# Ecogenomics/CheckM

Hardware: NVIDIA H100
Metric: genomes/hour (higher is better)
Workload: dtype int16 (SSV) / u8 (MSV) / int16 (Viterbi) / f32 (Forward, domain definition)

## Files before the change

### checkm_b200/_lib.py

```python
import ctypes as C
import os

_HERE = os.path.dirname(os.path.abspath(__file__))
LIB_PATH = os.environ.get("CKM_LIBRARY") or os.path.join(_HERE, "libckm.so")


class ModelInfo(C.Structure):
    _fields_ = [("name", C.c_char * 128), ("acc", C.c_char * 64), ("desc", C.c_char * 256), ("M", C.c_int32),
                ("has_ga", C.c_int32), ("has_tc", C.c_int32), ("has_nc", C.c_int32),
                ("ga", C.c_float * 2), ("tc", C.c_float * 2), ("nc", C.c_float * 2), ("evparam", C.c_float * 6),
                ("ga_d", C.c_double * 2), ("tc_d", C.c_double * 2), ("nc_d", C.c_double * 2)]


class Hit(C.Structure):
    _fields_ = [("bin", C.c_int32), ("seq", C.c_int32), ("model", C.c_int32), ("tlen", C.c_int32), ("qlen", C.c_int32),
                ("dom", C.c_int32), ("ndom", C.c_int32),
                ("hmm_from", C.c_int32), ("hmm_to", C.c_int32), ("ali_from", C.c_int32), ("ali_to", C.c_int32),
                ("env_from", C.c_int32), ("env_to", C.c_int32),
                ("full_score", C.c_float), ("full_bias", C.c_float), ("dom_score", C.c_float), ("dom_bias", C.c_float),
                ("acc", C.c_float),
                ("full_evalue", C.c_double), ("c_evalue", C.c_double), ("i_evalue", C.c_double),
                ("full_lnP", C.c_double), ("dom_lnP", C.c_double)]


class Stats(C.Structure):
    _fields_ = [("n_pairs", C.c_int64), ("n_cells", C.c_int64), ("n_ssv_cand", C.c_int64), ("n_past_msv", C.c_int64),
                ("n_past_bias", C.c_int64), ("n_past_vit", C.c_int64), ("n_past_fwd", C.c_int64),
                ("n_hits_seq", C.c_int64), ("n_domains", C.c_int64), ("n_reported", C.c_int64),
                ("ms_ssv", C.c_float), ("ms_msv", C.c_float), ("ms_bias", C.c_float), ("ms_vit", C.c_float),
                ("ms_fwd", C.c_float), ("ms_domdef", C.c_float), ("ms_total", C.c_float),
                ("kernel_launches", C.c_int64), ("n_vit_redo", C.c_int64), ("n_msv_exact", C.c_int64),
                ("n_queue_retries", C.c_int64)]


class QaRow(C.Structure):
    _fields_ = [("bin", C.c_int32), ("counts", C.c_int32 * 6), ("n_markers", C.c_int32), ("n_sets", C.c_int32),
                ("unique_hits", C.c_int32), ("multi_hits", C.c_int32),
                ("completeness", C.c_double), ("contamination", C.c_double)]


class MarkerHit(C.Structure):
    _fields_ = [("bin", C.c_int32), ("model", C.c_int32), ("seq_a", C.c_int32), ("seq_b", C.c_int32),
                ("target_length", C.c_int32), ("hmm_from", C.c_int32), ("hmm_to", C.c_int32),
                ("ali_from", C.c_int32), ("ali_to", C.c_int32), ("env_from", C.c_int32), ("env_to", C.c_int32),
                ("order", C.c_int32), ("src_row", C.c_int32), ("dict_key", C.c_int64)]


class ReduceOpts(C.Structure):
    _fields_ = [("ignore_thresholds", C.c_int32), ("skip_pseudogene", C.c_int32), ("skip_adjacent", C.c_int32),
                ("individual_markers", C.c_int32), ("evalue_threshold", C.c_double), ("evalue_exp10", C.c_int32),
                ("pad0", C.c_int32), ("evalue_mant", C.c_double), ("length_threshold", C.c_double),
                ("pseudogene_length", C.c_double)]


class ReduceMeta(C.Structure):
    _fields_ = [("is_pfam", C.c_void_p), ("is_tigr", C.c_void_p), ("clan", C.c_void_p),
                ("nest_off", C.c_void_p), ("nest_idx", C.c_void_p), ("has_cut", C.c_void_p), ("cutoffs", C.c_void_p), ("row_scores", C.c_void_p),
                ("scaffold_id", C.c_void_p), ("orf_num", C.c_void_p), ("name_rank", C.c_void_p),
                ("bin_set_off", C.c_void_p), ("set_marker_off", C.c_void_p), ("set_marker_idx", C.c_void_p)]


class BamFilter(C.Structure):
    _fields_ = [("all_reads", C.c_int32), ("min_qc", C.c_int32), ("min_align", C.c_double), ("max_edit", C.c_double)]


class OutlierIn(C.Structure):
    _fields_ = [("nseq", C.c_int64), ("nbins", C.c_int32), ("ntables", C.c_int32), ("bin_off", C.c_void_p),
                ("len", C.c_void_p), ("acgt", C.c_void_p), ("coding", C.c_void_p), ("sig_row", C.c_void_p),
                ("bin_gc_table", C.c_void_p), ("bin_cd_table", C.c_void_p), ("td_table", C.c_int32), ("pad", C.c_int32),
                ("table_off", C.c_void_p), ("table_key", C.c_void_p), ("table_lo", C.c_void_p), ("table_hi", C.c_void_p),
                ("binsig_in", C.c_void_p)]


class OutlierOut(C.Structure):
    _fields_ = [("bin_means", C.c_void_p), ("bin_sig", C.c_void_p), ("seq_values", C.c_void_p), ("seq_mask", C.c_void_p),
                ("kernel_ms", C.c_float * 3)]


SYMBOLS = ["ckm_init", "ckm_destroy", "ckm_last_error", "ckm_version", "ckm_device_name",
           "ckm_models_load", "ckm_models_count", "ckm_models_info", "ckm_models_find", "ckm_models_select",
           "ckm_models_write", "ckm_models_free", "ckm_digitize", "ckm_fasta_parse", "ckm_seqdb_create", "ckm_seqdb_free",
           "ckm_search", "ckm_search_per_bin", "ckm_hits_free", "ckm_align", "ckm_last_stats", "ckm_msv_scores",
           "ckm_filter_scores", "ckm_viterbi_scores", "ckm_write_domtblout", "ckm_reduce", "ckm_genome_check", "ckm_free", "ckm_allgather_qa", "ckm_nccl_unique_id",
           "ckm_nccl_comm_init", "ckm_nccl_comm_destroy", "ckm_fasta_scan_nt", "ckm_scaffold_stats",
           "ckm_kmer_counts", "ckm_kmer_columns", "ckm_format_kmer_profiles", "ckm_merge_pairs", "ckm_format_merger_rows",
           "ckm_bgzf_blocks", "ckm_bgzf_inflate", "ckm_bam_coverage", "ckm_bam_windows",
           "ckm_parse_kmer_profiles", "ckm_sigs_create", "ckm_sigs_free", "ckm_outlier_scores", "ckm_window_stats",
           "ckm_id_join", "ckm_format_unbinned"]

_lib = None


def lib():
    global _lib
    if _lib is not None:
        return _lib
    if not os.path.exists(LIB_PATH):
        raise ImportError("checkm_b200: %s is missing; run `python -c 'import __graft_entry__ as g; g.build()'` "
                          "(there is no CPU fallback)" % LIB_PATH)
    L = C.CDLL(LIB_PATH)
    vp, i32, i64, dbl = C.c_void_p, C.c_int32, C.c_int64, C.c_double
    L.ckm_last_error.restype = C.c_char_p
    L.ckm_version.restype = C.c_char_p
    L.ckm_init.argtypes = [C.c_int, C.POINTER(vp)]
    L.ckm_destroy.argtypes = [vp]
    L.ckm_destroy.restype = None
    L.ckm_device_name.argtypes = [vp, C.c_char_p, C.c_int]
    L.ckm_models_load.argtypes = [vp, C.c_char_p, C.POINTER(vp)]
    L.ckm_models_count.argtypes = [vp]
    L.ckm_models_info.argtypes = [vp, C.c_int, C.POINTER(ModelInfo)]
    L.ckm_models_find.argtypes = [vp, C.c_char_p]
    L.ckm_models_select.argtypes = [vp, C.POINTER(C.c_char_p), C.c_int, vp, C.POINTER(C.c_int)]
    L.ckm_models_write.argtypes = [vp, vp, C.c_int, C.c_char_p]
    L.ckm_models_free.argtypes = [vp]
    L.ckm_models_free.restype = None
    L.ckm_digitize.argtypes = [C.c_char_p, i64, vp]
    L.ckm_fasta_parse.argtypes = [C.c_char_p, i64, vp, vp, i32, vp, i64, C.POINTER(i32), C.POINTER(i64), C.POINTER(i64)]
    L.ckm_fasta_scan_nt.argtypes = [C.c_char_p, i64, vp, i64, vp, vp, i32, vp, i64, C.POINTER(i32), C.POINTER(i64), C.POINTER(i64)]
    L.ckm_scaffold_stats.argtypes = [vp, vp, i64, vp, vp, i32, vp, vp, vp, i64, C.POINTER(i64), C.POINTER(C.c_float)]
    L.ckm_kmer_counts.argtypes = [vp, vp, i64, vp, vp, i32, i32, vp, C.POINTER(C.c_float)]
    L.ckm_kmer_columns.argtypes = [i32, vp]
    L.ckm_format_kmer_profiles.argtypes = [vp, i32, i32, vp, vp, vp, i64, C.POINTER(i64)]
    L.ckm_merge_pairs.argtypes = [vp, vp, i32, i32, vp, dbl, dbl, dbl, dbl, vp, i64, C.POINTER(i64), C.POINTER(C.c_float)]
    L.ckm_format_merger_rows.argtypes = [vp, vp, i32, vp, vp, vp, vp, i64, vp, i64, C.POINTER(i64)]
    L.ckm_parse_kmer_profiles.argtypes = [C.c_char_p, i64, i32, i32, vp, vp, vp, i64, C.POINTER(i64)]
    L.ckm_sigs_create.argtypes = [vp, vp, i64, C.POINTER(vp)]
    L.ckm_sigs_free.argtypes = [vp]
    L.ckm_sigs_free.restype = None
    L.ckm_outlier_scores.argtypes = [vp, vp, C.POINTER(OutlierIn), C.POINTER(OutlierOut)]
    L.ckm_id_join.argtypes = [vp, C.c_char_p, i64, i32, vp, i64, vp, vp, vp, vp, vp, C.POINTER(i64), C.POINTER(i64),
                              C.POINTER(C.c_float)]
    L.ckm_format_unbinned.argtypes = [vp, vp, vp, vp, vp, vp, vp, i64, vp, i64, vp, i64, C.POINTER(i64), C.POINTER(i64)]
    L.ckm_window_stats.argtypes = [vp, vp, i64, vp, vp, i32, i64, vp, vp, vp, vp, C.POINTER(C.c_float)]
    L.ckm_bgzf_blocks.argtypes = [vp, i64, i64, vp, i64, C.POINTER(i64), C.POINTER(i64)]
    L.ckm_bgzf_inflate.argtypes = [vp, vp, i64, i64, vp, i64, vp, i64, C.POINTER(i64), C.POINTER(C.c_float)]
    L.ckm_bam_coverage.argtypes = [vp, vp, i64, i64, vp, i64, vp, vp, i64, i32, C.POINTER(BamFilter), vp, vp, C.POINTER(i64)]
    L.ckm_bam_windows.argtypes = [vp, vp, i64, i64, vp, i64, vp, vp, i64, i32, C.POINTER(BamFilter), vp, i64, vp, vp, vp, vp,
                                  C.POINTER(i64)]
    L.ckm_seqdb_create.argtypes = [vp, vp, vp, i32, vp, i32, C.POINTER(vp)]
    L.ckm_seqdb_free.argtypes = [vp]
    L.ckm_seqdb_free.restype = None
    L.ckm_search.argtypes = [vp, vp, vp, i32, vp, dbl, dbl, C.POINTER(C.POINTER(Hit)), C.POINTER(i64)]
    L.ckm_search_per_bin.argtypes = [vp, vp, vp, vp, vp, dbl, dbl, C.POINTER(C.POINTER(Hit)), C.POINTER(i64)]
    L.ckm_align.argtypes = [vp, vp, i32, vp, vp, vp]
    L.ckm_hits_free.argtypes = [C.POINTER(Hit)]
    L.ckm_hits_free.restype = None
    L.ckm_last_stats.argtypes = [vp, C.POINTER(Stats)]
    L.ckm_msv_scores.argtypes = [vp, vp, vp, i32, vp, vp]
    L.ckm_filter_scores.argtypes = [vp, vp, vp, i32, vp, vp, vp, vp, vp]
    L.ckm_viterbi_scores.argtypes = [vp, vp, vp, i32, vp, i32, vp]
    L.ckm_write_domtblout.argtypes = [vp, C.POINTER(Hit), i64, i32, i32, C.POINTER(C.c_char_p), C.POINTER(C.c_char_p),
                                      C.c_char_p]
    L.ckm_reduce.argtypes = [vp, i32, i32, i32, C.POINTER(Hit), i64, C.POINTER(ReduceOpts), C.POINTER(ReduceMeta),
                             C.POINTER(C.POINTER(QaRow)), C.POINTER(i32), C.POINTER(C.POINTER(MarkerHit)),
                             C.POINTER(i64)]
    L.ckm_genome_check.argtypes = [vp, i32, vp, vp, vp, i32, vp]
    L.ckm_free.argtypes = [vp]
    L.ckm_free.restype = None
    L.ckm_allgather_qa.argtypes = [vp, vp, vp, i32, i32, i32, vp, vp]
    L.ckm_nccl_unique_id.argtypes = [vp, i32]
    L.ckm_nccl_comm_init.argtypes = [vp, i32, i32, vp, C.POINTER(vp)]
    L.ckm_nccl_comm_destroy.argtypes = [vp]
    L.ckm_nccl_comm_destroy.restype = None
    _lib = L
    return L


class CkmError(RuntimeError):
    def __init__(self, code, msg):
        RuntimeError.__init__(self, "libckm error %d: %s" % (code, msg))
        self.code = code


def check(rc):
    if rc != 0:
        raise CkmError(rc, lib().ckm_last_error().decode(errors="replace"))
```

### checkm_b200/csrc/fwdback_blk.cuh

```cuda
#pragma once
#include "device_utils.cuh"
#include "engine.hpp"
#include "fwdback.cuh"

namespace ckm {

constexpr int BLK_LOOKAHEAD_MAXQ = 16;

template <int Q, bool TSMEM>
struct BlkModel {
  int M;
  const float *rfb;
  const float4 *tsm;
  float4 t0[TSMEM ? 1 : Q], t1[TSMEM ? 1 : Q];
  int lane;
  __device__ __forceinline__ float4 T0(int q) const { return TSMEM ? tsm[q * 32 + lane] : t0[TSMEM ? 0 : q]; }
  __device__ __forceinline__ float4 T1(int q) const { return TSMEM ? tsm[(Q + q) * 32 + lane] : t1[TSMEM ? 0 : q]; }
};

template <int Q, bool TSMEM>
__device__ __forceinline__ void blk_model_load(BlkModel<Q, TSMEM> &bm, const ModelScalars &ms, const float4 *tfb, const float *rfb,
                                               float4 *tsm, int lane) {
  bm.M = ms.M; bm.lane = lane;
  bm.rfb = rfb + ms.blk_off * 32 * KPAD + lane;
  bm.tsm = tsm;
  const float4 *src = tfb + ms.blk_off * 32 * 2;
  if (TSMEM) {
    __syncwarp();
    for (int q = 0; q < Q; ++q) { tsm[q * 32 + lane] = __ldg(src + (q * 32 + lane) * 2); tsm[(Q + q) * 32 + lane] = __ldg(src + (q * 32 + lane) * 2 + 1); }
    __syncwarp();
  } else {
#pragma unroll
    for (int q = 0; q < Q; ++q) { bm.t0[TSMEM ? 0 : q] = __ldg(src + (q * 32 + lane) * 2); bm.t1[TSMEM ? 0 : q] = __ldg(src + (q * 32 + lane) * 2 + 1); }
  }
}

template <int Q, bool TSMEM, bool FULL, bool STORE_D = true>
__device__ __forceinline__ float forward_blk(const BlkModel<Q, TSMEM> &bm, const uint8_t *__restrict__ res, int L, const Specials sp,
                                             float *xmx, float *full) {
  const int lane = bm.lane;
  float Mx[Q], Ix[Q], Dx[Q];
#pragma unroll
  for (int q = 0; q < Q; ++q) { Mx[q] = 0.0f; Ix[q] = 0.0f; Dx[q] = 0.0f; }
  if (FULL) {
#pragma unroll
    for (int z = 0; z < 3 * Q; ++z) full[z * 32 + lane] = 0.0f;
  }
  float xE = 0.0f, xN = 1.0f, xJ = 0.0f, xB = sp.nmove, xC = 0.0f, totscale = 0.0f;
  if (xmx != nullptr && lane == 0) { xmx[X_E] = xE; xmx[X_N] = xN; xmx[X_J] = xJ; xmx[X_B] = xB; xmx[X_C] = xC; xmx[X_SCALE] = 1.0f; }
  constexpr bool LA = (Q <= BLK_LOOKAHEAD_MAXQ);
  float ecur[Q];
  int xnext;
  if (LA) {
    const float *rp = bm.rfb + (size_t)((L >= 1) ? __ldg(res) : 0) * Q * 32;
#pragma unroll
    for (int q = 0; q < Q; ++q) ecur[q] = __ldg(rp + q * 32);
    xnext = (L >= 2) ? __ldg(res + 1) : 0;
  } else xnext = (L >= 1) ? __ldg(res) : 0;
  for (int i = 1; i <= L; ++i) {
    float enext[LA ? Q : 1];
    {
      const float *rp = bm.rfb + (size_t)xnext * Q * 32;
      if (LA) {
#pragma unroll
        for (int q = 0; q < Q; ++q) enext[LA ? q : 0] = __ldg(rp + q * 32);
        xnext = (i + 2 <= L) ? __ldg(res + i + 1) : 0;
      } else {
#pragma unroll
        for (int q = 0; q < Q; ++q) ecur[q] = __ldg(rp + q * 32);
        xnext = (i + 1 <= L) ? __ldg(res + i) : 0;
      }
    }
    float pm_in = __shfl_up_sync(0xffffffffu, Mx[Q - 1], 1), pi_in = __shfl_up_sync(0xffffffffu, Ix[Q - 1], 1), pd_in = __shfl_up_sync(0xffffffffu, Dx[Q - 1], 1);
    if (lane == 0) { pm_in = 0.0f; pi_in = 0.0f; pd_in = 0.0f; }
    float md[Q], esum = 0.0f;
#pragma unroll
    for (int q = Q - 1; q >= 0; --q) {
      const float4 t0 = bm.T0(q), t1 = bm.T1(q);
      const float pm = (q > 0) ? Mx[q - 1] : pm_in, pi = (q > 0) ? Ix[q - 1] : pi_in, pd = (q > 0) ? Dx[q - 1] : pd_in;
      float sv = xB * t0.x;
      sv += pm * t0.y;
      sv += pi * t0.z;
      sv += pd * t0.w;
      sv *= ecur[q];
      const float nI = Mx[q] * t1.y + Ix[q] * t1.z;
      md[q] = sv * t1.x;
      Mx[q] = sv; Ix[q] = nI;
      esum += sv;
    }
    float Bb = 0.0f, Tb = 1.0f;
#pragma unroll
    for (int q = 0; q < Q; ++q) { const float tdd = bm.T1(q).w; Bb = md[q] + Bb * tdd; Tb *= tdd; }
    float Bs = Bb, Ts = Tb;
#pragma unroll
    for (int o = 1; o < 32; o <<= 1) {
      const float Bl = __shfl_up_sync(0xffffffffu, Bs, o), Tl = __shfl_up_sync(0xffffffffu, Ts, o);
      if (lane >= o) { Bs = Bs + Bl * Ts; Ts = Ts * Tl; }
    }
    float d = __shfl_up_sync(0xffffffffu, Bs, 1);
    if (lane == 0) d = 0.0f;
#pragma unroll
    for (int q = 0; q < Q; ++q) {
      const bool in = (lane * Q + q + 1) <= bm.M;
      Dx[q] = in ? d : 0.0f;
      esum += Dx[q];
      d = md[q] + d * bm.T1(q).w;
    }
    xE = warp_sum_float(esum);
    xN = xN * sp.nloop;
    xC = (xC * sp.nloop) + (xE * sp.emove);
    xJ = (xJ * sp.nloop) + (xE * sp.eloop);
    xB = (xJ * sp.nmove) + (xN * sp.nmove);
    float scale = 1.0f;
    if (xE > 1.0e4f) {
      scale = xE;
      const float inv = __fdiv_rn(1.0f, xE);
      xN = __fdiv_rn(xN, xE); xC = __fdiv_rn(xC, xE); xJ = __fdiv_rn(xJ, xE); xB = __fdiv_rn(xB, xE);
#pragma unroll
      for (int q = 0; q < Q; ++q) { Mx[q] *= inv; Dx[q] *= inv; Ix[q] *= inv; }
      totscale += (float)log((double)xE);
      xE = 1.0f;
    }
    if (FULL) {
      float *fr = full + (size_t)i * 3 * Q * 32 + lane;
#pragma unroll
      for (int q = 0; q < Q; ++q) { fr[q * 32] = Mx[q]; if (STORE_D) fr[(Q + q) * 32] = Dx[q]; fr[(2 * Q + q) * 32] = Ix[q]; }
    }
    if (xmx != nullptr && lane == 0) {
      float *xr = xmx + (size_t)i * X_NX;
      xr[X_E] = xE; xr[X_N] = xN; xr[X_J] = xJ; xr[X_B] = xB; xr[X_C] = xC; xr[X_SCALE] = scale;
    }
    if (LA) {
#pragma unroll
      for (int q = 0; q < Q; ++q) ecur[q] = enext[LA ? q : 0];
    }
  }
  return totscale + (float)log((double)(xC * sp.nmove));
}

__device__ __forceinline__ void prefetch_l2(const void *p) { asm volatile("prefetch.global.L2 [%0];" ::"l"(p)); }
template <int Q, bool TSMEM, int MODE>
__device__ __forceinline__ void backward_blk(const BlkModel<Q, TSMEM> &bm, const uint8_t *__restrict__ res, int L, const Specials sp,
                                             const float *fxmx, float *bxmx, float *full) {
  const int lane = bm.lane, M = bm.M;
  float Mx[Q], Ix[Q], Dx[Q];
#pragma unroll
  for (int q = 0; q < Q; ++q) { Mx[q] = 0.0f; Ix[q] = 0.0f; Dx[q] = 0.0f; }
  float xC = 0.0f, xE = 0.0f, xJ = 0.0f, xN = 0.0f, xB = 0.0f;
  constexpr bool LA = (Q <= BLK_LOOKAHEAD_MAXQ);
  float ecur[Q];
#pragma unroll
  for (int q = 0; q < Q; ++q) ecur[q] = 0.0f;
  int xnext = (L >= 1) ? __ldg(res + L - 1) : 0;
  for (int i = L; i >= 0; --i) {
    float enext[LA ? Q : 1];
    if (LA) {
      const float *rp = bm.rfb + (size_t)xnext * Q * 32;
#pragma unroll
      for (int q = 0; q < Q; ++q) enext[LA ? q : 0] = __ldg(rp + q * 32);
      xnext = (i >= 2) ? __ldg(res + i - 2) : 0;
    } else if (i < L) {
      const float *rp = bm.rfb + (size_t)xnext * Q * 32;
#pragma unroll
      for (int q = 0; q < Q; ++q) ecur[q] = __ldg(rp + q * 32);
      xnext = (i >= 1) ? __ldg(res + i - 1) : 0;
    }
    if (MODE == 2 && i >= 3) {
      const float *fr = full + (size_t)(i - 2) * 3 * Q * 32;
      if (lane < Q) { prefetch_l2(fr + lane * 32); prefetch_l2(fr + (2 * Q + lane) * 32); }
    }
    float em[Q];
    if (i == L) {
      xC = sp.nmove; xE = xC * sp.emove; xB = 0.0f; xJ = 0.0f; xN = 0.0f;
#pragma unroll
      for (int q = 0; q < Q; ++q) em[q] = 0.0f;
    } else {
      float part = 0.0f;
#pragma unroll
      for (int q = 0; q < Q; ++q) { em[q] = Mx[q] * ecur[q]; part += em[q] * bm.T0(q).x; }
      xB = warp_sum_float(part);
      xC = xC * sp.nloop;
      xJ = (xB * sp.nmove) + (xJ * sp.nloop);
      xN = (xB * sp.nmove) + (xN * sp.nloop);
      xE = (xC * sp.emove) + (xJ * sp.eloop);
    }
    const float s = (i >= 1) ? fxmx[(size_t)i * X_NX + X_SCALE] : 1.0f;
    if (i >= 1) {
      const float inv = (s > 1.0f) ? __fdiv_rn(1.0f, s) : 1.0f;
      float em_next = __shfl_down_sync(0xffffffffu, em[0], 1);
      float4 tn_next;
      {
        const float4 mine = bm.T0(0);
        tn_next.x = 0.0f;
        tn_next.y = __shfl_down_sync(0xffffffffu, mine.y, 1); tn_next.z = __shfl_down_sync(0xffffffffu, mine.z, 1); tn_next.w = __shfl_down_sync(0xffffffffu, mine.w, 1);
      }
      if (lane == 31) { em_next = 0.0f; tn_next.y = 0.0f; tn_next.z = 0.0f; tn_next.w = 0.0f; }
      float cb[Q];
      float Bb = 0.0f, Tb = 1.0f;
#pragma unroll
      for (int q = Q - 1; q >= 0; --q) {
        const int k = lane * Q + q + 1;
        const float mnext = (q < Q - 1) ? em[q + 1] : em_next;
        const float tdm = (q < Q - 1) ? bm.T0(q + 1).w : tn_next.w;
        const bool in = (k <= M);
        cb[q] = in ? (xE + ((k < M) ? mnext * tdm : 0.0f)) : 0.0f;
        const float tdd = in ? bm.T1(q).w : 0.0f;
        Bb = cb[q] + Bb * tdd; Tb *= tdd;
      }
      float Bs = Bb, Ts = Tb;
#pragma unroll
      for (int o = 1; o < 32; o <<= 1) {
        const float Br = __shfl_down_sync(0xffffffffu, Bs, o), Tr = __shfl_down_sync(0xffffffffu, Ts, o);
        if (lane + o < 32) { Bs = Bs + Br * Ts; Ts = Ts * Tr; }
      }
      float dnext = __shfl_down_sync(0xffffffffu, Bs, 1);
      if (lane == 31) dnext = 0.0f;
      float nM[Q], nI[Q], nD[Q];
#pragma unroll
      for (int q = Q - 1; q >= 0; --q) {
        const int k = lane * Q + q + 1;
        const bool in = (k <= M);
        const float4 t1 = bm.T1(q);
        const float mnext = (q < Q - 1) ? em[q + 1] : em_next;
        const float4 tn = (q < Q - 1) ? bm.T0(q + 1) : tn_next;
        const float tmm = (k < M) ? tn.y : 0.0f, tim = (k < M) ? tn.z : 0.0f;
        const float inext = (i < L) ? Ix[q] : 0.0f;
        const float dv = in ? (cb[q] + dnext * t1.w) : 0.0f;
        float mv = xE + mnext * tmm + inext * t1.y + dnext * t1.x;
        float iv = mnext * tim + inext * t1.z;
        if (!in) { mv = 0.0f; iv = 0.0f; }
        nM[q] = mv * inv; nI[q] = iv * inv; nD[q] = dv * inv;
        dnext = dv;
      }
#pragma unroll
      for (int q = 0; q < Q; ++q) { Mx[q] = nM[q]; Ix[q] = nI[q]; Dx[q] = nD[q]; }
      if (s > 1.0f) { xE = __fdiv_rn(xE, s); xN = __fdiv_rn(xN, s); xJ = __fdiv_rn(xJ, s); xB = __fdiv_rn(xB, s); xC = __fdiv_rn(xC, s); }
    } else {
      xC = 0.0f; xJ = 0.0f; xE = 0.0f;
#pragma unroll
      for (int q = 0; q < Q; ++q) { Mx[q] = 0.0f; Ix[q] = 0.0f; Dx[q] = 0.0f; }
    }
    if (MODE == 1) {
      float *fr = full + (size_t)i * 3 * Q * 32 + lane;
#pragma unroll
      for (int q = 0; q < Q; ++q) { fr[q * 32] = Mx[q]; fr[(Q + q) * 32] = Dx[q]; fr[(2 * Q + q) * 32] = Ix[q]; }
    }
    if (MODE == 2 && i >= 1) {
      float *fr = full + (size_t)i * 3 * Q * 32 + lane;
      float fm[Q], fi[Q];
#pragma unroll
      for (int q = 0; q < Q; ++q) { fm[q] = fr[q * 32]; fi[q] = fr[(2 * Q + q) * 32]; }
#pragma unroll
      for (int q = 0; q < Q; ++q) { fr[q * 32] = fm[q] * Mx[q]; fr[(2 * Q + q) * 32] = fi[q] * Ix[q]; }
    }
    if (bxmx != nullptr && lane == 0) {
      float *xr = bxmx + (size_t)i * X_NX;
      xr[X_E] = xE; xr[X_N] = xN; xr[X_J] = xJ; xr[X_B] = xB; xr[X_C] = xC; xr[X_SCALE] = s;
    }
    if (LA) {
#pragma unroll
      for (int q = 0; q < Q; ++q) ecur[q] = enext[LA ? q : 0];
    }
  }
}

}
```

### checkm_b200/csrc/kernels_blk.cu

```cuda
#include "engine.hpp"
#include "device_utils.cuh"
#include "stages.hpp"
#include "fwdback.cuh"
#include "fwdback_blk.cuh"
#include "domdef_common.cuh"
#include "filter_common.cuh"

namespace ckm {

constexpr int BLK_WARPS = 4;

__host__ __device__ constexpr size_t blk_tsm_bytes(int Q) { return (size_t)Q * 32 * 2 * sizeof(float4); }

template <int Q, bool TSMEM>
__global__ void __launch_bounds__(BLK_WARPS * 32) fwd2_kernel(FilterParams p) {
  extern __shared__ __align__(16) uint8_t bsm[];
  const int lane = threadIdx.x & 31, warp = threadIdx.x >> 5;
  float4 *tsm = reinterpret_cast<float4 *>(bsm) + (size_t)warp * Q * 32 * 2;
  const int n = min(*p.in_count, p.in_cap);
  for (int c = blockIdx.x * BLK_WARPS + warp; c < n; c += gridDim.x * BLK_WARPS) {
    Candidate cd = p.in[c];
    const ModelScalars ms = p.ms[cd.model];
    if (ms.vq != Q) continue;
    const int s = cd.seq, L = p.len[s];
    BlkModel<Q, TSMEM> bm;
    blk_model_load<Q, TSMEM>(bm, ms, p.tfb, p.rfb, tsm, lane);
    const float fsc = forward_blk<Q, TSMEM, false>(bm, p.res + p.off[s], L, make_specials(L, true), nullptr, nullptr);
    fwd_verdict(p, cd, fsc, ms, lane);
  }
}

template <int Q, bool TSMEM>
__global__ void __launch_bounds__(BLK_WARPS * 32) regions2_kernel(DomdefParams p) {
  extern __shared__ __align__(16) uint8_t bsm[];
  const int lane = threadIdx.x & 31, warp = threadIdx.x >> 5;
  float4 *tsm = reinterpret_cast<float4 *>(bsm) + (size_t)warp * Q * 32 * 2;
  for (int idx = p.pair_begin + blockIdx.x * BLK_WARPS + warp; idx < p.pair_end; idx += gridDim.x * BLK_WARPS) {
    const int pi = p.pair_order[idx];
    const PairWork pw = p.pairs[pi];
    const ModelScalars ms = p.ms[pw.model];
    if (ms.vq != Q) continue;
    const int L = pw.L;
    BlkModel<Q, TSMEM> bm;
    blk_model_load<Q, TSMEM>(bm, ms, p.tfb, p.rfb, tsm, lane);
    const uint8_t *res = p.res + p.off[pw.seq];
    const Specials sp = make_specials(L, true);
    float *xf = p.xf + pw.row_off * X_NX, *xb = p.xb + pw.row_off * X_NX;
    forward_blk<Q, TSMEM, false>(bm, res, L, sp, xf, nullptr);
    __syncwarp();
    backward_blk<Q, TSMEM, 0>(bm, res, L, sp, xf, xb, nullptr);
    __syncwarp();
    regions_tail(p, pi, L, sp, xf, xb, p.btot + pw.row_off, p.etot + pw.row_off, p.mocc + pw.row_off, p.n2sc + pw.row_off, lane);
    __syncwarp();
  }
}

template <int Q> struct BlockedLayout {
  const float *F; const float4 *tfb; int M;
  static __device__ __forceinline__ int at(int k) { return ((k - 1) % Q) * 32 + (k - 1) / Q; }
  __device__ __forceinline__ float cell(int row, int plane, int k) const { return F[((int64_t)row * 3 + plane) * (Q * 32) + at(k)]; }
  __device__ __forceinline__ float4 t0(int k) const { return __ldg(tfb + at(k) * 2); }
  __device__ __forceinline__ float4 t1(int k) const { return __ldg(tfb + at(k) * 2 + 1); }
  __device__ __forceinline__ void row_best(int row, int lane, float &bm, int &bk, float &bd, int &bdk) const {
    const float *dpc = F + (int64_t)row * 3 * (Q * 32) + lane;
    if constexpr (Q <= 12) {
#pragma unroll
      for (int q = 0; q < Q; ++q) {
        const int kk = lane * Q + q + 1;
        if (kk <= M) {
          const float v = dpc[q * 32]; if (v >= bm) { bm = v; bk = kk; }
          const float w = dpc[(Q + q) * 32]; if (w > bd) { bd = w; bdk = kk; }
        }
      }
    } else {
#pragma unroll 4
      for (int q = 0; q < Q; ++q) {
        const int kk = lane * Q + q + 1;
        if (kk <= M) { const float v = dpc[q * 32]; if (v >= bm) { bm = v; bk = kk; } }
      }
#pragma unroll 4
      for (int q = 0; q < Q; ++q) {
        const int kk = lane * Q + q + 1;
        if (kk <= M) { const float w = dpc[(Q + q) * 32]; if (w > bd) { bd = w; bdk = kk; } }
      }
    }
  }
};

template <int Q, bool TSMEM>
__global__ void __launch_bounds__(BLK_WARPS * 32) envelope2_kernel(DomdefParams p) {
  extern __shared__ __align__(16) uint8_t bsm[];
  const int lane = threadIdx.x & 31, warp = threadIdx.x >> 5;
  float4 *tsm = reinterpret_cast<float4 *>(bsm) + (size_t)warp * Q * 32 * 2;
  float *null2 = reinterpret_cast<float *>(bsm + (TSMEM ? BLK_WARPS * blk_tsm_bytes(Q) : 0)) + warp * 32;
  constexpr int QW = Q * 32;
  for (int idx = p.env_begin + blockIdx.x * BLK_WARPS + warp; idx < p.env_end; idx += gridDim.x * BLK_WARPS) {
    const int ei = p.env_order[idx];
    const Envelope env = p.envs[ei];
    const PairWork pw = p.pairs[env.pair];
    const ModelScalars ms = p.ms[pw.model];
    if (ms.vq != Q) continue;
    BlkModel<Q, TSMEM> bm;
    blk_model_load<Q, TSMEM>(bm, ms, p.tfb, p.rfb, tsm, lane);
    const int M = ms.M, Ld = env.j - env.i + 1;
    const uint8_t *res = p.res + p.off[pw.seq] + (env.i - 1);
    const Specials sp = make_specials(pw.L, false);
    const int64_t mat = (int64_t)(Ld + 1) * 3 * QW;
    float *F = p.scratch + env.scratch_off, *Bm = F;
    float *xf = F + mat, *xb = xf + (int64_t)(Ld + 1) * X_NX, *pps = xb + (int64_t)(Ld + 1) * X_NX;
    float *xo = xf;
    float *n2sc = p.n2sc + pw.row_off;
    const float envsc = forward_blk<Q, TSMEM, true, false>(bm, res, Ld, sp, xf, F);
    __syncwarp();
    backward_blk<Q, TSMEM, 2>(bm, res, Ld, sp, xf, xb, F);
    __syncwarp();
    const float scaleproduct = __fdiv_rn(1.0f, xb[X_N]);
    float em[Q], ein[Q];
#pragma unroll
    for (int q = 0; q < Q; ++q) { em[q] = 0.0f; ein[q] = 0.0f; }
    for (int r = 1; r <= Ld; ++r) {
      if (r + 2 <= Ld && lane < Q) {
        const float *fn = F + (int64_t)(r + 2) * 3 * QW;
        prefetch_l2(fn + lane * 32); prefetch_l2(fn + (2 * Q + lane) * 32);
      }
      const float totr = scaleproduct * xf[(int64_t)r * X_NX + X_SCALE];
      const float *fr = F + (int64_t)r * 3 * QW + lane;
      float vm[Q], vi[Q];
#pragma unroll
      for (int q = 0; q < Q; ++q) { vm[q] = fr[q * 32]; vi[q] = fr[(2 * Q + q) * 32]; }
#pragma unroll
      for (int q = 0; q < Q; ++q) {
        const float pm = vm[q] * totr, pi = vi[q] * totr;
        em[q] = (r == 1) ? pm : em[q] + pm;
        ein[q] = (r == 1) ? pi : ein[q] + pi;
      }
    }
    special_posteriors(sp, xf, xb, scaleproduct, pps, Ld, lane);
    const bool range_err = isinf(scaleproduct);
    if (!range_err && !env.null2_done) {
      const float norm = __fdiv_rn(1.0f, (float)Ld);
      const float xfactor = special_xfactor(pps, Ld, norm, lane);
#pragma unroll
      for (int q = 0; q < Q; ++q) { em[q] *= norm; ein[q] *= norm; }
      for (int x = 0; x < K; ++x) {
        const float *rp = bm.rfb + (size_t)x * QW;
        float part = 0.0f;
#pragma unroll
        for (int q = 0; q < Q; ++q) { part += em[q] * __ldg(rp + q * 32); part += ein[q]; }
        part = warp_sum_float(part);
        if (lane == 0) null2[x] = part + xfactor;
      }
      null2_finish(null2, n2sc, res, env, lane);
    }
    float oasc = 0.0f;
    const float NINF = -INFINITY;
    if (!range_err) {
      float oM[Q], oI[Q], oD[Q];
#pragma unroll
      for (int q = 0; q < Q; ++q) { oM[q] = NINF; oI[q] = NINF; oD[q] = NINF; }
#pragma unroll
      for (int z = 0; z < 3 * Q; ++z) Bm[z * 32 + lane] = NINF;
      OaSpecials os(sp);
      os.store(xo, lane);
      for (int r = 1; r <= Ld; ++r) {
        if (r + 2 <= Ld && lane < Q) {
          const float *fn = F + (int64_t)(r + 2) * 3 * QW;
          prefetch_l2(fn + lane * 32); prefetch_l2(fn + (2 * Q + lane) * 32);
        }
        const float totr = scaleproduct * xf[(int64_t)r * X_NX + X_SCALE];
        const float *ppr = F + (int64_t)r * 3 * QW + lane;
        float *orow = Bm + (int64_t)r * 3 * QW + lane;
        float ppm[Q], ppi[Q];
#pragma unroll
        for (int q = 0; q < Q; ++q) { ppm[q] = ppr[q * 32]; ppi[q] = ppr[(2 * Q + q) * 32]; }
        float pm_in = __shfl_up_sync(0xffffffffu, oM[Q - 1], 1), pi_in = __shfl_up_sync(0xffffffffu, oI[Q - 1], 1), pd_in = __shfl_up_sync(0xffffffffu, oD[Q - 1], 1);
        if (lane == 0) { pm_in = NINF; pi_in = NINF; pd_in = NINF; }
        float a[Q]; bool ps[Q];
        float emax = NINF;
#pragma unroll
        for (int q = Q - 1; q >= 0; --q) {
          const float4 t0 = bm.T0(q), t1 = bm.T1(q);
          const bool in = (lane * Q + q + 1) <= M;
          const float pm = (q > 0) ? oM[q - 1] : pm_in, pi = (q > 0) ? oI[q - 1] : pi_in, pd = (q > 0) ? oD[q - 1] : pd_in;
          float sv = (t0.x > 0.0f) ? os.B : 0.0f;
          sv = fmaxf(sv, (t0.y > 0.0f) ? pm : 0.0f);
          sv = fmaxf(sv, (t0.z > 0.0f) ? pi : 0.0f);
          sv = fmaxf(sv, (t0.w > 0.0f) ? pd : 0.0f);
          sv += ppm[q] * totr;
          if (!in) sv = NINF;
          const float nI = in ? fmaxf((t1.y > 0.0f) ? oM[q] : 0.0f, (t1.z > 0.0f) ? oI[q] : 0.0f) + ppi[q] * totr : NINF;
          a[q] = (t1.x > 0.0f) ? sv : 0.0f;
          ps[q] = (t1.w > 0.0f);
          if (!in) { a[q] = NINF; ps[q] = true; }
          if (!ps[q]) a[q] = fmaxf(a[q], 0.0f);
          oM[q] = sv; oI[q] = nI;
          emax = fmaxf(emax, sv);
        }
        float A = NINF; bool pass = true;
#pragma unroll
        for (int q = 0; q < Q; ++q) { if (ps[q]) { A = fmaxf(a[q], A); } else { A = a[q]; pass = false; } }
        float As = A; bool Ps = pass;
#pragma unroll
        for (int o = 1; o < 32; o <<= 1) {
          const float Al = __shfl_up_sync(0xffffffffu, As, o);
          const int pl = __shfl_up_sync(0xffffffffu, (int)Ps, o);
          if (lane >= o && Ps) { As = fmaxf(As, Al); Ps = (pl != 0); }
        }
        float d = __shfl_up_sync(0xffffffffu, As, 1);
        if (lane == 0) d = NINF;
#pragma unroll
        for (int q = 0; q < Q; ++q) {
          const bool in = (lane * Q + q + 1) <= M;
          oD[q] = in ? d : NINF;
          emax = fmaxf(emax, oD[q]);
          d = ps[q] ? fmaxf(a[q], d) : a[q];
        }
#pragma unroll
        for (int o = 16; o > 0; o >>= 1) emax = fmaxf(emax, __shfl_xor_sync(0xffffffffu, emax, o));
        os.row(sp, pps + r * 3, emax);
#pragma unroll
        for (int q = 0; q < Q; ++q) { orow[q * 32] = oM[q]; orow[(Q + q) * 32] = oD[q]; orow[(2 * Q + q) * 32] = oI[q]; }
        os.store(xo + (int64_t)r * X_NX, lane);
      }
      oasc = os.C;
    }
    __syncwarp();
    OaTrace tr;
    if (!range_err) tr = oa_traceback(BlockedLayout<Q>{Bm, p.tfb + ms.blk_off * 64, M}, p, pw, env, sp, xo, pps, Ld, M, lane);
    write_domain(p, env, n2sc, tr, envsc, oasc, lane);
    __syncwarp();
  }
}

template <class P, class KF>
static int launch_blk(KF kern, const char *name, int Q, bool tsmem, const P &p, int grid, size_t extra, cudaStream_t st) {
  return launch_kernel(kern, name, grid, BLK_WARPS * 32, (tsmem ? BLK_WARPS * blk_tsm_bytes(Q) : 0) + extra, st, p);
}
int launch_fwd2(const FilterParams &p, int cls, int grid, cudaStream_t st) {
  return with_class(cls, [&](auto Q, auto TSMEM) { return launch_blk(fwd2_kernel<Q, TSMEM>, "fwd2_kernel", Q, TSMEM, p, grid, 0, st); });
}
int launch_regions2(const DomdefParams &p, int cls, int grid, cudaStream_t st) {
  return with_class(cls, [&](auto Q, auto TSMEM) { return launch_blk(regions2_kernel<Q, TSMEM>, "regions2_kernel", Q, TSMEM, p, grid, 0, st); });
}
int launch_envelopes2(const DomdefParams &p, int cls, int grid, cudaStream_t st) {
  return with_class(cls, [&](auto Q, auto TSMEM) {
    return launch_blk(envelope2_kernel<Q, TSMEM>, "envelope2_kernel", Q, TSMEM, p, grid, BLK_WARPS * 32 * sizeof(float), st);
  });
}

}
```

### checkm_b200/csrc/kernels_vitp.cu

```cuda
#include "engine.hpp"
#include "device_utils.cuh"
#include "stages.hpp"
#include "filter_common.cuh"

namespace ckm {

constexpr uint32_t VP_FLOORW = 0xD800D800u;
constexpr int      VP_FLOOR  = -10240;
constexpr uint32_t VP_TFLOORW = 0xC000C000u;

__device__ __forceinline__ int vp_lo(uint32_t w) { return (int)(int16_t)(w & 0xffffu); }
__device__ __forceinline__ int vp_hi(uint32_t w) { return (int)w >> 16; }

__global__ void vit_count_kernel(FilterParams p, int32_t *cnt) {
  const int n = min(*p.in_count, p.in_cap);
  for (int i = blockIdx.x * blockDim.x + threadIdx.x; i < n; i += gridDim.x * blockDim.x) {
    const Candidate cd = p.in[i];
    if (!(cd.P > p.F2)) filter_pass(p, cd, 4);
    else if (p.ms[cd.model].vq == 0) vit_redo(p, cd);
    else atomicAdd(cnt + cd.model, 1);
  }
}

__global__ void __launch_bounds__(1024) vit_scan_kernel(FilterParams p, int32_t nmodels, const int32_t *cnt, int32_t *off, int32_t *choff) {
  __shared__ int ws[2][32];
  const int lane = threadIdx.x & 31, warp = threadIdx.x >> 5;
  int run_pairs = 0, run_chunks = 0;
  for (int c = 0; c < N_BLK_CLASSES; ++c) {
    if (threadIdx.x == 0) p.vit_cls_chunks[c] = run_chunks;
    for (int b = 0; b < nmodels; b += 1024) {
      const int m = b + threadIdx.x;
      const int v = (m < nmodels && blk_class(p.ms[m].vq) == c) ? cnt[m] : 0, h = (v + VITP_CHUNK - 1) / VITP_CHUNK;
      int sv = v, sh = h;
#pragma unroll
      for (int o = 1; o < 32; o <<= 1) {
        const int a = __shfl_up_sync(0xffffffffu, sv, o), d = __shfl_up_sync(0xffffffffu, sh, o);
        if (lane >= o) { sv += a; sh += d; }
      }
      if (lane == 31) { ws[0][warp] = sv; ws[1][warp] = sh; }
      __syncthreads();
      if (warp == 0) {
        int tv = ws[0][lane], th = ws[1][lane];
#pragma unroll
        for (int o = 1; o < 32; o <<= 1) {
          const int a = __shfl_up_sync(0xffffffffu, tv, o), d = __shfl_up_sync(0xffffffffu, th, o);
          if (lane >= o) { tv += a; th += d; }
        }
        ws[0][lane] = tv; ws[1][lane] = th;
      }
      __syncthreads();
      if (v > 0) {
        off[m] = run_pairs + (warp ? ws[0][warp - 1] : 0) + sv - v;
        choff[m] = run_chunks + (warp ? ws[1][warp - 1] : 0) + sh - h;
      }
      run_pairs += ws[0][31]; run_chunks += ws[1][31];
      __syncthreads();
    }
  }
  if (threadIdx.x == 0) p.vit_cls_chunks[N_BLK_CLASSES] = run_chunks;
}

__global__ void vit_scatter_kernel(FilterParams p, const int32_t *cnt, int32_t *fill, const int32_t *off, const int32_t *choff) {
  const int n = min(*p.in_count, p.in_cap);
  for (int i = blockIdx.x * blockDim.x + threadIdx.x; i < n; i += gridDim.x * blockDim.x) {
    const int m = p.in[i].model;
    if (!(p.in[i].P > p.F2) || p.ms[m].vq == 0) continue;
    const int r = atomicAdd(fill + m, 1), pos = off[m] + r;
    p.vit_idx[pos] = i;
    if (r % VITP_CHUNK == 0) p.vit_chunks[choff[m] + r / VITP_CHUNK] = make_int2(pos, off[m] + min(r + VITP_CHUNK, cnt[m]));
  }
}

int launch_vit_group(const FilterParams &p, int32_t nmodels, int32_t *ws, int grid, cudaStream_t st) {
  int32_t *cnt = ws, *fill = ws + nmodels, *off = ws + 2 * (size_t)nmodels, *choff = ws + 3 * (size_t)nmodels;
  cudaError_t e = cudaMemsetAsync(ws, 0, sizeof(int32_t) * 2 * (size_t)nmodels, st);
  if (e != cudaSuccess) return cuda_fail(e, "cudaMemsetAsync(vit groups)");
  vit_count_kernel<<<grid, 256, 0, st>>>(p, cnt);
  vit_scan_kernel<<<1, 1024, 0, st>>>(p, nmodels, cnt, off, choff);
  vit_scatter_kernel<<<grid, 256, 0, st>>>(p, cnt, fill, off, choff);
  e = cudaGetLastError();
  return e == cudaSuccess ? CKM_OK : cuda_fail(e, "vit grouping launch");
}

constexpr int VITP_THREADS = 128;

__host__ __device__ constexpr int vitp_smem_bytes(int W, bool tsmem) { return KPAD * W * 32 * 4 + (tsmem ? W * 64 * 16 : 0); }
__host__ __device__ constexpr int vitp_min_blocks(int W) { return W <= 4 ? 4 : (W <= 10 ? 3 : 2); }

template <int W, bool TSMEM>
__global__ void __launch_bounds__(VITP_THREADS, vitp_min_blocks(W)) vitp_kernel(FilterParams p, int cls) {
  extern __shared__ __align__(16) uint4 vsm[];
  __shared__ int s_chunk, s_next;
  __shared__ ModelScalars s_ms;
  uint32_t *esm = reinterpret_cast<uint32_t *>(vsm);
  uint4 *tws = vsm + KPAD * W * 8;
  const int lane = threadIdx.x & 31;
  const uint32_t sel = (lane == 0) ? 0x1054u : 0x3210u;
  const int c0 = p.vit_cls_chunks[cls], nch = p.vit_cls_chunks[cls + 1] - c0;
  for (;;) {
    __syncthreads();
    if (threadIdx.x == 0) {
      const int k = atomicAdd(p.vit_work + cls, 1);
      s_chunk = k;
      if (k < nch) {
        s_next = p.vit_chunks[c0 + k].x;
        s_ms = p.ms[p.in[p.vit_idx[s_next]].model];
      }
    }
    __syncthreads();
    const int k = s_chunk;
    if (k >= nch) break;
    const int2 ch = p.vit_chunks[c0 + k];
    const ModelScalars &ms = s_ms;
    {
      const uint4 *esrc = reinterpret_cast<const uint4 *>(p.rwp + ms.blk_off * 32 * (KPAD / 2));
      for (int z = threadIdx.x; z < KPAD * W * 8; z += VITP_THREADS) vsm[z] = __ldg(esrc + z);
      if (TSMEM) {
        const uint4 *tsrc = p.twp + ms.blk_off * 32;
        for (int z = threadIdx.x; z < W * 64; z += VITP_THREADS) tws[(z & 1) * (W * 32) + (z >> 1)] = __ldg(tsrc + z);
      }
    }
    uint4 tr0[TSMEM ? 1 : W], tr1[TSMEM ? 1 : W];
    if (!TSMEM) {
      const uint4 *tsrc = p.twp + ms.blk_off * 32;
#pragma unroll
      for (int w = 0; w < W; ++w) { tr0[TSMEM ? 0 : w] = __ldg(tsrc + (w * 32 + lane) * 2); tr1[TSMEM ? 0 : w] = __ldg(tsrc + (w * 32 + lane) * 2 + 1); }
    }
#define TR0(w) (TSMEM ? tws[(w) * 32 + lane] : tr0[TSMEM ? 0 : (w)])
#define TR1(w) (TSMEM ? tws[W * 32 + (w) * 32 + lane] : tr1[TSMEM ? 0 : (w)])
    __syncthreads();
    const uint32_t *erow = esm + lane;
    const int ddbound = ms.ddbound_w, cap = 32767 - (int)ms.vit_emax;
    const int e_move = ms.xw_e_move, e_loop = ms.xw_e_loop;
    for (;;) {
      int j = 0;
      if (lane == 0) j = atomicAdd(&s_next, 1);
      j = __shfl_sync(0xffffffffu, j, 0);
      if (j >= ch.y) break;
      const Candidate *cin = p.in + p.vit_idx[j];
      const int s = cin->seq, L = p.len[s];
      bool redo = false;
      const int tmove = p.tmove_w[s];
      const int cost = -tmove - (int)ms.vit_tbm + 64;
      const bool c1 = (cost - (int)ms.xw_e_loop <= 22528) && (cost <= 22240);
      const bool c1p = (cost - (int)ms.xw_e_loop <= 16384);
      redo = !c1;
      float vsc = 0.0f;
      if (!redo) {
        uint32_t Mx[W], Ix[W], Dx[W];
#pragma unroll
        for (int w = 0; w < W; ++w) { Mx[w] = VP_FLOORW; Ix[w] = VP_FLOORW; Dx[w] = VP_FLOORW; }
        int xN = ms.base_w, xB = xN + tmove, xJ = -32768, xC = -32768;
        const uint32_t *rp = reinterpret_cast<const uint32_t *>(p.res + p.off[s]);
        const int nw = (L + 3) >> 2;
        uint32_t wcur = (nw > 0) ? __ldg(rp) : 0u;
        bool stop = false;
        for (int q = 0; q < nw && !stop; ++q) {
          const uint32_t wnext = (q + 1 < nw) ? __ldg(rp + q + 1) : 0u;
#pragma unroll
          for (int rr = 0; rr < 4; ++rr) {
            if (q * 4 + rr >= L) { stop = true; break; }
            const uint32_t *ew = erow + ((wcur >> (8 * rr)) & 0xffu) * (W * 32);
            const uint32_t shM = __shfl_sync(0xffffffffu, Mx[W - 1], (lane + 31) & 31);
            const uint32_t shI = __shfl_sync(0xffffffffu, Ix[W - 1], (lane + 31) & 31);
            const uint32_t shD = __shfl_sync(0xffffffffu, Dx[W - 1], (lane + 31) & 31);
            const uint32_t pm0 = __byte_perm(shM, VP_FLOORW, sel), pi0 = __byte_perm(shI, VP_FLOORW, sel), pd0 = __byte_perm(shD, VP_FLOORW, sel);
            const uint32_t xBw = __byte_perm((uint32_t)xB, 0u, 0x1010u);
            uint32_t md[W];
            uint32_t xEw = VP_FLOORW, dmw = VP_FLOORW;
#pragma unroll
            for (int w = W - 1; w >= 0; --w) {
              const uint32_t pm = (w > 0) ? Mx[w - 1] : pm0, pi = (w > 0) ? Ix[w - 1] : pi0, pd = (w > 0) ? Dx[w - 1] : pd0;
              const uint4 t0 = TR0(w), t1 = TR1(w);
              uint32_t sv = __viaddmax_s16x2(xBw, t0.x, VP_FLOORW);
              sv = __viaddmax_s16x2(pm, t0.y, sv);
              sv = __viaddmax_s16x2(pi, t0.z, sv);
              sv = __viaddmax_s16x2(pd, t0.w, sv);
              sv = __viaddmax_s16x2(sv, ew[w * 32], VP_FLOORW);
              const uint32_t nI = __viaddmax_s16x2(Ix[w], t1.z, __viaddmax_s16x2(Mx[w], t1.y, VP_FLOORW));
              md[w] = __viaddmax_s16x2(sv, t1.x, VP_FLOORW);
              Mx[w] = sv; Ix[w] = nI;
            }
#pragma unroll
            for (int w = 0; w + 1 < W; w += 2) { xEw = __vimax3_s16x2(xEw, Mx[w], Mx[w + 1]); dmw = __vimax3_s16x2(dmw, md[w], md[w + 1]); }
            if (W & 1) { xEw = __vimax3_s16x2(xEw, Mx[W - 1], Mx[W - 1]); dmw = __vimax3_s16x2(dmw, md[W - 1], md[W - 1]); }
            const int xE = __reduce_max_sync(0xffffffffu, max(vp_lo(xEw), vp_hi(xEw)));
            if (xE >= cap) { redo = true; stop = true; break; }
            xC = max(xC, xE + e_move);
            xJ = max(xJ, xE + e_loop);
            xB = max(xJ + tmove, xN + tmove);
            const int Dmax = __reduce_max_sync(0xffffffffu, max(vp_lo(dmw), vp_hi(dmw)));
            if (Dmax + ddbound > xB) {
              if (!c1p) { redo = true; stop = true; break; }
              uint32_t Bb = VP_FLOORW, Tb = 0u;
#pragma unroll
              for (int w = 0; w < W; ++w) { const uint32_t tdd = TR1(w).w; Bb = __viaddmax_s16x2(Bb, tdd, md[w]); Tb = __viaddmax_s16x2(Tb, __vimax3_s16x2(tdd, VP_TFLOORW, VP_TFLOORW), VP_TFLOORW); }
              uint32_t Bs = Bb, Ts = Tb;
#pragma unroll
              for (int o = 1; o < 32; o <<= 1) {
                const uint32_t Bl = __shfl_up_sync(0xffffffffu, Bs, o), Tl = __shfl_up_sync(0xffffffffu, Ts, o);
                if (lane >= o) { Bs = __viaddmax_s16x2(Bl, Ts, Bs); Ts = __viaddmax_s16x2(Ts, Tl, VP_TFLOORW); }
              }
              uint32_t din = __shfl_up_sync(0xffffffffu, Bs, 1), Tex = __shfl_up_sync(0xffffffffu, Ts, 1);
              if (lane == 0) { din = VP_FLOORW; Tex = 0u; }
              const uint32_t lowexit = __shfl_sync(0xffffffffu, Bs, 31);
              const uint32_t dmid = __byte_perm(lowexit, VP_FLOORW, 0x1054u);
              din = __viaddmax_s16x2(dmid, Tex, din);
              uint32_t d = din;
#pragma unroll
              for (int w = 0; w < W; ++w) { Dx[w] = d; d = __viaddmax_s16x2(d, TR1(w).w, md[w]); }
            } else {
              const uint32_t shd = __shfl_sync(0xffffffffu, md[W - 1], (lane + 31) & 31);
#pragma unroll
              for (int w = W - 1; w >= 1; --w) Dx[w] = md[w - 1];
              Dx[0] = __byte_perm(shd, VP_FLOORW, sel);
            }
          }
          wcur = wnext;
        }
        if (!redo && xC <= VP_FLOOR + e_move) redo = true;
        if (!redo) vsc = vit_vsc(xC, tmove, ms);
      }
      Candidate cd = *cin;
      if (redo) {
        if (lane == 0) vit_redo(p, cd);
        continue;
      }
      if (vit_verdict(p, cd, vsc, ms, lane) && lane == 0) filter_pass(p, cd, 4);
    }
#undef TR0
#undef TR1
  }
}

__global__ void all_pairs_kernel(Candidate *out, int32_t *count, const int32_t *slot_model, int32_t nslots, int32_t nseq) {
  const int64_t n = (int64_t)nslots * nseq;
  for (int64_t i = blockIdx.x * (int64_t)blockDim.x + threadIdx.x; i < n; i += (int64_t)gridDim.x * blockDim.x) {
    Candidate cd;
    cd.seq = (int32_t)(i % nseq); cd.model = slot_model[i / nseq]; cd.usc = 0.0f; cd.filtersc = 0.0f; cd.vitsc = 0.0f; cd.fwdsc = 0.0f; cd.P = 1.0;
    out[i] = cd;
  }
  if (blockIdx.x == 0 && threadIdx.x == 0) *count = (int32_t)n;
}
int launch_all_pairs(Candidate *out, int32_t *count, const int32_t *slot_model, int32_t nslots, int32_t nseq, cudaStream_t st) {
  return launch_kernel(all_pairs_kernel, "all_pairs_kernel", 592, 256, 0, st, out, count, slot_model, nslots, nseq);
}

int launch_vitp(const FilterParams &p, int cls, int grid, cudaStream_t st) {
  return with_class(cls, [&](auto Q, auto TSMEM) {
    return launch_kernel(vitp_kernel<Q / 2, TSMEM>, "vitp_kernel", grid, VITP_THREADS, vitp_smem_bytes(Q / 2, TSMEM), st, p, cls);
  });
}

}
```

### checkm_b200/csrc/search.cu

```cuda
#include <algorithm>
#include <atomic>
#include <chrono>
#include <cstdio>
#include <cmath>
#include <cstdlib>
#include <cstring>
#include <memory>
#include <vector>
#include "engine.hpp"
#include "stages.hpp"
#include "pool.hpp"

using namespace ckm;

namespace ckm {

std::atomic<int> g_live_engines{0};
thread_local ckm_engine *g_pool_engine = nullptr;
thread_local int g_pool_next = 0;
constexpr int X_NX_HOST = 6;
struct EnsembleJob;
int ensembles_launch(ckm_engine *e, const ckm_models *m, DomdefParams &p, const std::vector<PairWork> &pairs,
                     const std::vector<Region> &regs, const std::vector<int> &multi_idx, const std::vector<EnsembleCaps> &caps,
                     cudaStream_t st, EnsembleJob **job_out);
int ensembles_collect(EnsembleJob *job, cudaStream_t st, std::vector<std::vector<Envelope>> &out, std::vector<EnsembleCaps> &grow, int *n_over);
void ensembles_abandon(EnsembleJob *job, cudaStream_t st);
enum { CTR_UNIT4 = 0, CTR_UNIT8, CTR_UNIT16, CTR_UNIT32, CTR_CAND, CTR_MSV, CTR_BIAS, CTR_VIT, CTR_FWD, CTR_ENV, CTR_DOM, CTR_VREDO, CTR_SSVRES, CTR_VWORK = 16 , CTR_N = 32 };
enum { EV_SSV = 0, EV_MSV, EV_BIAS, EV_VIT, EV_FWD, EV_CASCADE_END, EV_DOMDEF, EV_END, EV_CALL };

static int64_t env_scratch_budget() {
  if (const char *v = std::getenv("CKM_ENV_SCRATCH_MB")) {
    char *end = nullptr;
    const long long mb = std::strtoll(v, &end, 10);
    if (end != v && *end == '\0' && mb > 0) return (int64_t)std::min<long long>(mb, (long long)1 << 30) * ((int64_t)1 << 20) / (int64_t)sizeof(float);
  }
  size_t free_b = 0, total_b = 0;
  cudaMemGetInfo(&free_b, &total_b);
  const size_t neng = (size_t)std::max(1, g_live_engines.load());
  return (int64_t)std::min<size_t>(total_b * 4 / 10 / neng, (size_t)56 << 30) / (int64_t)sizeof(float);
}
struct SearchKnobs { bool blk, vitp, ssv_resolve, trace; int ens_first; int64_t env_budget; };
static SearchKnobs read_knobs(bool envelopes) {
  auto starts = [](const char *name, char c) { const char *v = std::getenv(name); return v != nullptr && v[0] == c; };
  SearchKnobs k;
  k.blk = !starts("CKM_BLK", '0');
  k.vitp = k.blk && !starts("CKM_VITP", '0');
  k.ssv_resolve = !starts("CKM_SSV_RESOLVE", '0');
  k.trace = starts("CKM_TRACE", '1');
  const char *ens = std::getenv("CKM_ENS_FIRST");
  k.ens_first = ens == nullptr ? -1 : (ens[0] == '0' ? 0 : 1);
  k.env_budget = envelopes ? env_scratch_budget() : 0;
  return k;
}
struct Trace {
  bool on; std::chrono::steady_clock::time_point t0, last;
  explicit Trace(bool on_) : on(on_) { t0 = last = std::chrono::steady_clock::now(); }
  void mark(const char *what) {
    if (!on) return;
    const auto now = std::chrono::steady_clock::now();
    std::fprintf(stderr, "[ckm trace] %-28s +%8.3f ms  (%9.3f)\n", what, std::chrono::duration<double, std::milli>(now - last).count(),
                 std::chrono::duration<double, std::milli>(now - t0).count());
    last = now;
  }
};

static int cls_of(int M, bool use_blk) { return use_blk ? blk_class(vq_of(M)) : N_BLK_CLASSES; }

static int fan_out(ckm_engine *e) {
  CKM_CUDA(cudaEventRecord(e->fan_ev, e->stream));
  for (auto &s : e->cls) CKM_CUDA(cudaStreamWaitEvent(s, e->fan_ev, 0));
  return CKM_OK;
}
static int fan_in(ckm_engine *e) {
  for (int c = 0; c < ckm_engine::NCLS; ++c) {
    CKM_CUDA(cudaEventRecord(e->cls_ev[c], e->cls[c]));
    CKM_CUDA(cudaStreamWaitEvent(e->stream, e->cls_ev[c], 0));
  }
  return CKM_OK;
}

template <class P> static int per_class(ckm_engine *e, const P &p, int (*blocked)(const P &, int, int, cudaStream_t), int blk_per_sm,
                                        int (*unblocked)(const P &, int, cudaStream_t), int per_sm, bool widest_first = false) {
  const int nsm = e->prop.multiProcessorCount;
  int rc;
  if ((rc = fan_out(e))) return rc;
  for (int i = 0; i < ckm_engine::NCLS; ++i) {
    const int c = widest_first ? ckm_engine::NCLS - 1 - i : i;
    if (c == N_BLK_CLASSES) rc = unblocked ? unblocked(p, nsm * per_sm, e->cls[c]) : CKM_OK;
    else rc = p.use_blk ? blocked(p, c, nsm * blk_per_sm, e->cls[c]) : CKM_OK;
    if (rc) return rc;
  }
  return fan_in(e);
}
template <class Launch> static int launch_class_runs(ckm_engine *e, const std::vector<int32_t> &order, const std::vector<int8_t> &cls, size_t b0, size_t b1, Launch launch) {
  const int nsm = e->prop.multiProcessorCount;
  int rc;
  if ((rc = fan_out(e))) return rc;
  while (b0 < b1) {
    size_t r1 = b0; const int c = cls[order[b0]];
    while (r1 < b1 && cls[order[r1]] == c) ++r1;
    const int cnt = (int)(r1 - b0);
    const int grid = c < N_BLK_CLASSES ? std::min(nsm * 8, (cnt + 3) / 4) : std::min(nsm * 4, (cnt + FWD_WARPS - 1) / FWD_WARPS);
    if ((rc = launch(c, (int32_t)b0, (int32_t)r1, grid, e->cls[c]))) return rc;
    e->stats.kernel_launches++;
    b0 = r1;
  }
  return CKM_OK;
}

struct ActiveMasks { DevBuf tile_active, model_active, model_slot; bool all_active = true; };
static FilterParams filter_params(const ckm_models *m, const ckm_seqdb *db, ActiveMasks &am) {
  FilterParams p{};
  p.res = db->d_res; p.off = db->d_off; p.len = db->d_len; p.lenA = db->d_lenA; p.lenB = db->d_lenB; p.tmove_w = db->d_tmove_w;
  p.ms = m->d_scalars; p.bias_eo = m->d_bias_eo; p.rwv = m->d_rwv; p.twv = m->d_twv; p.rfv = m->d_rfv; p.tfv = m->d_tfv;
  p.twb = m->d_twb; p.rwb = m->d_rwb; p.tfb = m->d_tfb; p.rfb = m->d_rfb; p.twp = m->d_twp; p.rwp = m->d_rwp;
  p.row_elems = ((m->maxM + 31) / 32) * 32 + 64;
  p.F1 = 0.02; p.F2 = 1e-3; p.F3 = 1e-5;
  p.model_slot = am.model_slot.as<int32_t>(); p.nseq = db->nseq;
  return p;
}

static DomdefParams domdef_params(const ckm_models *m, const ckm_seqdb *db, const SearchKnobs &k) {
  DomdefParams p{};
  p.res = db->d_res; p.off = db->d_off; p.nullsc = db->d_nullsc; p.ms = m->d_scalars; p.rfv = m->d_rfv; p.tfv = m->d_tfv;
  p.row_elems = ((m->maxM + 31) / 32) * 32 + 64;
  p.tfb = m->d_tfb; p.rfb = m->d_rfb; p.use_blk = k.blk ? 1 : 0;
  return p;
}
static void fill_filter_stats(ckm_engine *e, int64_t n_pairs, const int32_t *ctr, unsigned long long cells, int stages) {
  ckm_stats &s = e->stats;
  s.n_pairs = n_pairs; s.n_cells = (int64_t)cells;
  s.n_ssv_cand = (int64_t)ctr[CTR_CAND] + ctr[CTR_SSVRES]; s.n_msv_exact = ctr[CTR_CAND]; s.n_past_msv = ctr[CTR_MSV]; s.n_past_bias = ctr[CTR_BIAS];
  s.n_past_vit = ctr[CTR_VIT]; s.n_past_fwd = ctr[CTR_FWD]; s.n_vit_redo = ctr[CTR_VREDO];
  float *ms[] = {&s.ms_ssv, &s.ms_msv, &s.ms_bias, &s.ms_vit, &s.ms_fwd};
  for (int i = 0; i < stages; ++i) cudaEventElapsedTime(ms[i], e->ev[EV_SSV + i], e->ev[EV_SSV + i + 1]);
}
static std::vector<float> &logsum_table() {
  static std::vector<float> t = [] {
    std::vector<float> v(16000);
    for (int i = 0; i < 16000; ++i) v[i] = (float)std::log(1.0 + std::exp((double)-i / 1000.0));
    return v;
  }();
  return t;
}

static int build_masks(const ckm_models *m, const ckm_seqdb *db, const int32_t *model_idx, int32_t nmodels,
                       const int64_t *bin_model_offsets, ActiveMasks &am, std::vector<int32_t> &slot_of_model, cudaStream_t st) {
  const int ndb = (int)m->models.size(), nbins = db->nbins, ntiles = (int)m->tiles.size();
  slot_of_model.assign(ndb, -1);
  bool all = (bin_model_offsets == nullptr) && (model_idx == nullptr || nmodels == ndb);
  if (model_idx == nullptr) { for (int i = 0; i < ndb; ++i) slot_of_model[i] = i; }
  else if (bin_model_offsets == nullptr) {
    for (int i = 0; i < nmodels; ++i) {
      if (model_idx[i] < 0 || model_idx[i] >= ndb) { set_error("model index out of range"); return CKM_EINVAL; }
      if (slot_of_model[model_idx[i]] >= 0) { set_error("duplicate model index in query list"); return CKM_EINVAL; }
      slot_of_model[model_idx[i]] = i;
    }
    if (all) for (int i = 0; i < ndb; ++i) if (slot_of_model[i] < 0) all = false;
  }
  am.all_active = all;
  int rc;
  if ((rc = am.model_slot.alloc(sizeof(int32_t) * ndb))) return rc;
  CKM_CUDA(cudaMemcpyAsync(am.model_slot.p, slot_of_model.data(), sizeof(int32_t) * ndb, cudaMemcpyHostToDevice, st));
  if (all) return CKM_OK;
  std::vector<uint8_t> ma((size_t)nbins * ndb, 0), ta((size_t)nbins * ntiles, 0);
  for (int b = 0; b < nbins; ++b) {
    if (bin_model_offsets == nullptr) {
      for (int i = 0; i < nmodels; ++i) ma[(size_t)b * ndb + model_idx[i]] = 1;
    } else {
      for (int64_t i = bin_model_offsets[b]; i < bin_model_offsets[b + 1]; ++i) {
        if (model_idx[i] < 0 || model_idx[i] >= ndb) { set_error("model index out of range"); return CKM_EINVAL; }
        if (ma[(size_t)b * ndb + model_idx[i]]) { set_error("duplicate model index in the query list of bin " + std::to_string(b)); return CKM_EINVAL; }
        ma[(size_t)b * ndb + model_idx[i]] = 1;
      }
    }
    for (int t = 0; t < ntiles; ++t) {
      const TileDesc &td = m->tiles[t];
      uint8_t any = 0;
      for (int j = 0; j < td.nmodels; ++j) any |= ma[(size_t)b * ndb + m->tile_models[td.first_model + j].model];
      ta[(size_t)b * ntiles + t] = any;
    }
  }
  if ((rc = am.model_active.alloc(ma.size()))) return rc;
  if ((rc = am.tile_active.alloc(ta.size()))) return rc;
  CKM_CUDA(cudaMemcpyAsync(am.model_active.p, ma.data(), ma.size(), cudaMemcpyHostToDevice, st));
  CKM_CUDA(cudaMemcpyAsync(am.tile_active.p, ta.data(), ta.size(), cudaMemcpyHostToDevice, st));
  CKM_CUDA(cudaStreamSynchronize(st));
  return CKM_OK;
}
struct Stage1 {
  DevBuf cand, pass, bnd, glist, cells;
  int32_t cand_cap = 0, pass_cap = 0;
};
constexpr int64_t QUEUE_MAX = (int64_t)1 << 30;
constexpr int QUEUE_ATTEMPTS = 3;
static int32_t queue_cap(int64_t n_pairs, int64_t divisor, int attempt) {
  int64_t want = n_pairs / divisor + 65536;
  for (int a = 0; a < attempt && want < n_pairs; ++a) want *= 8;
  return (int32_t)std::min<int64_t>(std::min<int64_t>(n_pairs, QUEUE_MAX), std::max<int64_t>((int64_t)1 << 16, want));
}

static int run_stage1(ckm_engine *e, const SearchKnobs &k, const ckm_models *m, const ckm_seqdb *db, ActiveMasks &am, int64_t n_pairs,
                      Stage1 &s1, int32_t *xj_dense, int attempt = 0) {
  cudaStream_t st = e->stream;
  int rc;
  s1.cand_cap = queue_cap(n_pairs, 6, attempt);
  const int64_t n_bypass = (int64_t)m->ssv_bypass.size() * db->nseq;
  s1.cand_cap = (int32_t)std::min<int64_t>(QUEUE_MAX, (int64_t)s1.cand_cap + n_bypass);
  s1.pass_cap = queue_cap(n_pairs, 12, attempt);
  if ((rc = s1.cand.alloc(sizeof(int2) * (size_t)s1.cand_cap))) return rc;
  if ((rc = s1.pass.alloc(sizeof(Candidate) * (size_t)s1.pass_cap))) return rc;
  if ((rc = s1.cells.alloc(sizeof(unsigned long long)))) return rc;
  CKM_CUDA(cudaMemsetAsync(e->d_counters, 0, CTR_N * sizeof(int32_t), st));
  CKM_CUDA(cudaMemsetAsync(s1.cells.p, 0, sizeof(unsigned long long), st));
  const int nsm = e->prop.multiProcessorCount;
  bool need_bnd = false;
  for (int nt : m->chain_ntiles) need_bnd |= (nt > 1);
  const int64_t bnd_stride = ((int64_t)db->maxL + 31) / 16 * 16;
  if (need_bnd) { if ((rc = s1.bnd.alloc((size_t)nsm * SSV_WARPS_HOST * 2 * bnd_stride * sizeof(int16_t)))) return rc; }
  std::vector<int32_t> gl[4];
  for (size_t g = 0; g < m->groups.size(); ++g) gl[m->groups[g].J == 4 ? 0 : (m->groups[g].J == 8 ? 1 : (m->groups[g].J == 16 ? 2 : 3))].push_back((int32_t)g);
  std::vector<int32_t> flat;
  size_t goff[4];
  for (int c = 0; c < 4; ++c) { goff[c] = flat.size(); flat.insert(flat.end(), gl[c].begin(), gl[c].end()); }
  if ((rc = s1.glist.alloc(sizeof(int32_t) * std::max<size_t>(flat.size(), 1)))) return rc;
  if (!flat.empty()) CKM_CUDA(cudaMemcpyAsync(s1.glist.p, flat.data(), sizeof(int32_t) * flat.size(), cudaMemcpyHostToDevice, st));
  CKM_CUDA(cudaStreamSynchronize(st));

  CKM_CUDA(cudaEventRecord(e->ev[EV_SSV], st));
  SsvParams sp{};
  sp.res = db->d_res; sp.off = db->d_off; sp.len = db->d_len; sp.bin = db->d_bin;
  sp.msvB = db->d_msvB; sp.tjb = db->d_tjb; sp.order = db->d_order;
  sp.nseq = db->nseq; sp.seq_chunk = 128; sp.nchunks = (db->nseq + sp.seq_chunk - 1) / sp.seq_chunk;
  sp.groups = m->d_groups; sp.tiles = m->d_tiles; sp.tile_models = m->d_tile_models; sp.tile_blob = m->d_tile_blob;
  sp.chain_first_tile = m->d_chain_first_tile; sp.chain_ntiles = m->d_chain_ntiles;
  sp.tile_active = am.all_active ? nullptr : am.tile_active.as<uint8_t>();
  sp.model_active = am.all_active ? nullptr : am.model_active.as<uint8_t>();
  sp.ntiles = (int32_t)m->tiles.size(); sp.nmodels = (int32_t)m->models.size();
  sp.cand = s1.cand.as<int2>(); sp.cand_count = e->d_counters + CTR_CAND; sp.cand_cap = s1.cand_cap;
  sp.bnd = need_bnd ? s1.bnd.as<int16_t>() : nullptr; sp.bnd_stride = bnd_stride;
  sp.cells = s1.cells.as<unsigned long long>();
  sp.resolve = k.ssv_resolve ? 1 : 0;
  sp.ms = m->d_scalars; sp.nullsc = db->d_nullsc;
  sp.pass = s1.pass.as<Candidate>(); sp.pass_count = e->d_counters + CTR_MSV; sp.pass_cap = s1.pass_cap;
  sp.resolved_count = e->d_counters + CTR_SSVRES;
  sp.xj_dense = xj_dense; sp.model_slot = am.model_slot.as<int32_t>();
  sp.F1 = 0.02;
  const int Js[4] = {4, 8, 16, 32};
  for (int c = 0; c < 4; ++c) {
    if (gl[c].empty() || db->nseq == 0) continue;
    sp.group_list = s1.glist.as<int32_t>() + goff[c]; sp.ngroups = (int32_t)gl[c].size();
    sp.unit_counter = e->d_counters + CTR_UNIT4 + c;
    int64_t maxbytes = 0;
    for (int g : gl[c]) maxbytes = std::max<int64_t>(maxbytes, m->groups[g].table_bytes);
    const int64_t units = (int64_t)sp.ngroups * sp.nchunks;
    const int grid = (int)std::min<int64_t>(nsm, units);
    if ((rc = launch_ssv(Js[c], sp, grid, (size_t)maxbytes, st))) return rc;
    e->stats.kernel_launches++;
  }
  if (!m->ssv_bypass.empty()) {
    if ((rc = launch_ssv_bypass(m->d_ssv_bypass, (int32_t)m->ssv_bypass.size(), db->nseq, db->d_len, db->d_bin,
                                am.all_active ? nullptr : am.model_active.as<uint8_t>(), (int32_t)m->models.size(),
                                s1.cand.as<int2>(), e->d_counters + CTR_CAND, s1.cand_cap, st))) return rc;
    e->stats.kernel_launches++;
  }
  CKM_CUDA(cudaEventRecord(e->ev[EV_MSV], st));
  MsvParams p{};
  p.res = db->d_res; p.off = db->d_off; p.len = db->d_len; p.nullsc = db->d_nullsc; p.tjb = db->d_tjb;
  p.ms = m->d_scalars; p.rbv = m->d_rbv; p.rmb = m->d_rmb;
  p.cand = s1.cand.as<int2>(); p.cand_count = e->d_counters + CTR_CAND; p.cand_cap = s1.cand_cap;
  p.out = s1.pass.as<Candidate>(); p.out_count = e->d_counters + CTR_MSV; p.out_cap = s1.pass_cap;
  p.xj_dense = xj_dense; p.model_slot = am.model_slot.as<int32_t>(); p.nseq = db->nseq;
  p.row_bytes = (m->maxM + 2 + 15) / 16 * 16;
  p.F1 = 0.02;
  p.use_blk = k.blk ? 1 : 0;
  if ((rc = per_class(e, p, launch_msv2, 16, launch_msv_exact, 4))) return rc;
  e->stats.kernel_launches += 1 + (p.use_blk ? N_BLK_CLASSES : 0);
  CKM_CUDA(cudaEventRecord(e->ev[EV_BIAS], st));
  return CKM_OK;
}

static int run_viterbi(ckm_engine *e, const ckm_models *m, FilterParams &p, bool packed, DevBuf &grp) {
  int rc;
  if (packed) {
    const int nm = (int)m->models.size();
    const size_t nchunks = (size_t)p.in_cap / VITP_CHUNK + nm + 1;
    const size_t words = 4 * (size_t)nm + 16 + ((size_t)p.in_cap + 1) / 2 * 2;
    if ((rc = grp.alloc(sizeof(int32_t) * words + sizeof(int2) * nchunks))) return rc;
    int32_t *ws = grp.as<int32_t>();
    p.vit_cls_chunks = ws + 4 * (size_t)nm;
    p.vit_idx = p.vit_cls_chunks + 16;
    p.vit_chunks = reinterpret_cast<int2 *>(ws + words);
    p.vit_work = e->d_counters + CTR_VWORK;
    if ((rc = launch_vit_group(p, nm, ws, e->prop.multiProcessorCount * 8, e->stream))) return rc;
    if ((rc = per_class<FilterParams>(e, p, launch_vitp, 8, nullptr, 0))) return rc;
    e->stats.kernel_launches += 3;
    p.in = p.redo; p.in_count = p.redo_count; p.in_cap = p.redo_cap;
  }
  return per_class(e, p, launch_vit2, 8, launch_vit, 4);
}
struct Stage2 {
  DevBuf a, b, redo, vgrp;
  int32_t cap = 0;
};
static int run_stage2(ckm_engine *e, const SearchKnobs &k, const ckm_models *m, const ckm_seqdb *db, ActiveMasks &am, Stage1 &s1, Stage2 &s2,
                      float *d_filtersc, float *d_vit, float *d_fwd, uint8_t *d_passed) {
  cudaStream_t st = e->stream;
  int rc;
  s2.cap = s1.pass_cap;
  if ((rc = s2.a.alloc(sizeof(Candidate) * (size_t)s2.cap))) return rc;
  if ((rc = s2.b.alloc(sizeof(Candidate) * (size_t)s2.cap))) return rc;
  if ((rc = s2.redo.alloc(sizeof(Candidate) * (size_t)s2.cap))) return rc;
  const int nsm = e->prop.multiProcessorCount;
  FilterParams p = filter_params(m, db, am);
  p.redo = s2.redo.as<Candidate>(); p.redo_count = e->d_counters + CTR_VREDO; p.redo_cap = s2.cap;
  p.use_blk = k.blk ? 1 : 0;
  p.dense_filtersc = d_filtersc; p.dense_vit = d_vit; p.dense_fwd = d_fwd; p.dense_passed = d_passed;
  p.in = s1.pass.as<Candidate>(); p.in_count = e->d_counters + CTR_MSV; p.in_cap = s1.pass_cap;
  p.out = s2.a.as<Candidate>(); p.out_count = e->d_counters + CTR_BIAS; p.out_cap = s2.cap;
  if ((rc = launch_bias(p, nsm * 8, st))) return rc;
  CKM_CUDA(cudaEventRecord(e->ev[EV_VIT], st));
  p.in = s2.a.as<Candidate>(); p.in_count = e->d_counters + CTR_BIAS; p.in_cap = s2.cap;
  p.out = s2.b.as<Candidate>(); p.out_count = e->d_counters + CTR_VIT; p.out_cap = s2.cap;
  if ((rc = run_viterbi(e, m, p, k.vitp, s2.vgrp))) return rc;
  CKM_CUDA(cudaEventRecord(e->ev[EV_FWD], st));
  p.in = s2.b.as<Candidate>(); p.in_count = e->d_counters + CTR_VIT; p.in_cap = s2.cap;
  p.out = s2.a.as<Candidate>(); p.out_count = e->d_counters + CTR_FWD; p.out_cap = s2.cap;
  if ((rc = per_class(e, p, launch_fwd2, 8, launch_fwd, 4, true))) return rc;
  CKM_CUDA(cudaEventRecord(e->ev[EV_CASCADE_END], st));
  e->stats.kernel_launches += 3 + (k.vitp ? N_BLK_CLASSES : 0) + (p.use_blk ? 2 * N_BLK_CLASSES : 0);
  return CKM_OK;
}

static int64_t envelope_need(const ckm_models *m, const PairWork &pw, const Envelope &en, bool use_blk) {
  const int64_t Ld = en.j - en.i + 1, Mpad = ((m->models[pw.model].M + 1) + 31) / 32 * 32 + 32;
  const int64_t vq = use_blk ? vq_of(m->models[pw.model].M) : 0;
  const int64_t width = vq ? 32 * vq : Mpad;
  return (vq ? 1 : 2) * (Ld + 1) * 3 * width + (Ld + 1) * 15 + 64;
}
static int run_envelope_waves(ckm_engine *e, const ckm_models *m, const std::vector<PairWork> &pairs, DomdefParams &p, int64_t budget,
                              DevBuf &scratch, std::vector<Envelope> &ev, DevBuf &d_ev, DevBuf &d_ord, bool leave_last) {
  if (ev.empty()) return CKM_OK;
  cudaStream_t st = e->stream;
  int rc;
  std::vector<int64_t> need(ev.size());
  std::vector<int8_t> ecls(ev.size());
  for (size_t i = 0; i < ev.size(); ++i) {
    const PairWork &pw = pairs[ev[i].pair];
    need[i] = envelope_need(m, pw, ev[i], p.use_blk != 0);
    ecls[i] = (int8_t)cls_of(m->models[pw.model].M, p.use_blk != 0);
  }
  budget = std::max<int64_t>(budget, *std::max_element(need.begin(), need.end()));
  if ((rc = d_ev.alloc(sizeof(Envelope) * ev.size())) || (rc = d_ord.alloc(sizeof(int32_t) * ev.size()))) return rc;
  std::vector<int32_t> eorder(ev.size());
  for (size_t w0 = 0, w1; w0 < ev.size(); w0 = w1) {
    int64_t tot = 0;
    for (w1 = w0; w1 < ev.size() && (w1 == w0 || tot + need[w1] <= budget); ++w1) { ev[w1].scratch_off = tot; tot += need[w1]; }
    if (sizeof(float) * (size_t)tot > scratch.bytes && (rc = scratch.alloc(sizeof(float) * (size_t)tot))) return rc;
    for (size_t i = w0; i < w1; ++i) eorder[i] = (int32_t)i;
    std::stable_sort(eorder.begin() + w0, eorder.begin() + w1, [&](int32_t a, int32_t b) { return ecls[a] != ecls[b] ? ecls[a] > ecls[b] : need[a] > need[b]; });
    CKM_CUDA(cudaMemcpyAsync(d_ev.as<Envelope>() + w0, ev.data() + w0, sizeof(Envelope) * (w1 - w0), cudaMemcpyHostToDevice, st));
    CKM_CUDA(cudaMemcpyAsync(d_ord.as<int32_t>() + w0, eorder.data() + w0, sizeof(int32_t) * (w1 - w0), cudaMemcpyHostToDevice, st));
    p.envs = d_ev.as<Envelope>(); p.env_order = d_ord.as<int32_t>(); p.scratch = scratch.as<float>();
    if ((rc = launch_class_runs(e, eorder, ecls, w0, w1, [&](int c, int32_t b0, int32_t b1, int grid, cudaStream_t s) -> int {
          p.env_begin = b0; p.env_end = b1; return c < N_BLK_CLASSES ? launch_envelopes2(p, c, grid, s) : launch_envelopes(p, grid, s); }))) return rc;
    CKM_CUDA(cudaStreamSynchronize(st));
    if (w1 < ev.size() || !leave_last) { if ((rc = fan_in(e))) return rc; CKM_CUDA(cudaStreamSynchronize(st)); }
  }
  return CKM_OK;
}

struct QueryPlan { ActiveMasks am; bool per_bin = false; std::vector<std::vector<int32_t>> qorder; int64_t n_pairs = 0; };
static int plan_queries(const ckm_models *m, const ckm_seqdb *db, const int32_t *model_idx, int32_t nmodels, const int64_t *bin_model_offsets, QueryPlan &q, cudaStream_t st) {
  const int ndb = (int)m->models.size();
  if (model_idx == nullptr && bin_model_offsets == nullptr) nmodels = ndb;
  std::vector<int32_t> slot;
  int rc = build_masks(m, db, model_idx, nmodels, bin_model_offsets, q.am, slot, st);
  if (rc) return rc;
  q.per_bin = bin_model_offsets != nullptr;
  if (q.per_bin) {
    q.qorder.assign(db->nbins, std::vector<int32_t>(ndb, -1));
    for (int b = 0; b < db->nbins; ++b) {
      for (int64_t i = bin_model_offsets[b]; i < bin_model_offsets[b + 1]; ++i) q.qorder[b][model_idx[i]] = (int32_t)(i - bin_model_offsets[b]);
      q.n_pairs += (int64_t)db->bin_nseq[b] * (bin_model_offsets[b + 1] - bin_model_offsets[b]);
    }
  } else {
    q.qorder.emplace_back(std::move(slot));
    q.n_pairs = (int64_t)db->nseq * nmodels;
  }
  return CKM_OK;
}

static int run_cascade(ckm_engine *e, const SearchKnobs &k, const ckm_models *m, const ckm_seqdb *db, ActiveMasks &am, int64_t n_pairs, Stage1 &s1, Stage2 &s2, int32_t *ctr) {
  cudaStream_t st = e->stream;
  unsigned long long cells = 0;
  int rc;
  for (int attempt = 0; attempt < QUEUE_ATTEMPTS; ++attempt) {
    if (attempt > 0) e->stats.n_queue_retries++;
    if ((rc = run_stage1(e, k, m, db, am, std::max<int64_t>(n_pairs, 1), s1, nullptr, attempt))) return rc;
    if ((rc = run_stage2(e, k, m, db, am, s1, s2, nullptr, nullptr, nullptr, nullptr))) return rc;
    CKM_CUDA(cudaMemcpyAsync(ctr, e->d_counters, sizeof(int32_t) * CTR_N, cudaMemcpyDeviceToHost, st));
    CKM_CUDA(cudaMemcpyAsync(&cells, s1.cells.p, sizeof(cells), cudaMemcpyDeviceToHost, st));
    CKM_CUDA(cudaStreamSynchronize(st));
    const bool over = ctr[CTR_CAND] > s1.cand_cap || ctr[CTR_MSV] > s1.pass_cap || ctr[CTR_BIAS] > s2.cap || ctr[CTR_VIT] > s2.cap || ctr[CTR_FWD] > s2.cap ||
                      ctr[CTR_VREDO] > s2.cap;
    if (!over) { fill_filter_stats(e, n_pairs, ctr, cells, 5); return CKM_OK; }
    if (s1.cand_cap >= std::min<int64_t>(n_pairs, QUEUE_MAX) && s1.pass_cap >= std::min<int64_t>(n_pairs, QUEUE_MAX)) break;
  }
  set_error("candidate queue overflow in the filter cascade: more than 2^30 candidate pairs in one batch; search fewer bins per call");
  return CKM_ECAPACITY;
}

static int sorted_pairs(const ckm_seqdb *db, const Candidate *d_fwd_list, int npairs, std::vector<PairWork> &pairs, int64_t &rows) {
  std::vector<Candidate> fl((size_t)npairs);
  if (npairs) CKM_CUDA(cudaMemcpy(fl.data(), d_fwd_list, sizeof(Candidate) * fl.size(), cudaMemcpyDeviceToHost));
  std::sort(fl.begin(), fl.end(), [](const Candidate &a, const Candidate &b) { return a.seq != b.seq ? a.seq < b.seq : a.model < b.model; });
  pairs.assign((size_t)npairs, PairWork{});
  rows = 0;
  for (int i = 0; i < npairs; ++i) {
    PairWork &pw = pairs[i];
    pw.seq = fl[i].seq; pw.model = fl[i].model; pw.L = db->len[pw.seq];
    pw.first_dom = 0; pw.ndom_slots = 0; pw.fwdsc = fl[i].fwdsc; pw.filtersc = fl[i].filtersc; pw.usc = fl[i].usc;
    pw.row_off = rows; rows += pw.L + 1;
  }
  return CKM_OK;
}
struct DomainStage {
  DomdefParams p{};
  DevBuf dpairs, dxf, dxb, dvec, dtbl, dregions, dporder, ddoms, dhits, dscratch, denvs, deorder, denvs2, deorder2;
  std::vector<Region> regs;
  std::vector<DomainOut> doms; std::vector<HitOut> hout;
};
static int run_regions(ckm_engine *e, const SearchKnobs &k, const ckm_models *m, const ckm_seqdb *db, const std::vector<PairWork> &pairs, int64_t rows, DomainStage &D, Trace &tr) {
  cudaStream_t st = e->stream;
  const int npairs = (int)pairs.size();
  const size_t rws = (size_t)std::max<int64_t>(rows, 1);
  int rc;
  if ((rc = D.dpairs.alloc(sizeof(PairWork) * pairs.size())) || (rc = D.dxf.alloc(sizeof(float) * rws * X_NX_HOST)) || (rc = D.dxb.alloc(sizeof(float) * rws * X_NX_HOST)) ||
      (rc = D.dvec.alloc(sizeof(float) * rws * 4)) || (rc = D.dtbl.alloc(sizeof(float) * 16000))) return rc;
  const int region_cap = npairs * 8 + 1024;
  if ((rc = D.dregions.alloc(sizeof(Region) * (size_t)region_cap))) return rc;
  CKM_CUDA(cudaMemcpyAsync(D.dpairs.p, pairs.data(), sizeof(PairWork) * pairs.size(), cudaMemcpyHostToDevice, st));
  CKM_CUDA(cudaMemcpyAsync(D.dtbl.p, logsum_table().data(), sizeof(float) * 16000, cudaMemcpyHostToDevice, st));
  CKM_CUDA(cudaMemsetAsync(e->d_counters + CTR_ENV, 0, sizeof(int32_t), st));
  DomdefParams &p = D.p = domdef_params(m, db, k);
  p.pairs = D.dpairs.as<PairWork>(); p.npairs = npairs;
  p.xf = D.dxf.as<float>(); p.xb = D.dxb.as<float>();
  p.btot = D.dvec.as<float>(); p.etot = p.btot + rws; p.mocc = p.etot + rws; p.n2sc = p.mocc + rws;
  p.regions = D.dregions.as<Region>(); p.region_count = e->d_counters + CTR_ENV; p.region_cap = region_cap;
  p.logsum_tbl = D.dtbl.as<float>();
  std::vector<int32_t> order((size_t)npairs);
  std::vector<int8_t> pcls((size_t)npairs);
  for (int i = 0; i < npairs; ++i) { order[i] = i; pcls[i] = (int8_t)cls_of(m->models[pairs[i].model].M, p.use_blk != 0); }
  std::stable_sort(order.begin(), order.end(), [&](int32_t a, int32_t b) { return pcls[a] != pcls[b] ? pcls[a] > pcls[b] : pairs[a].L > pairs[b].L; });
  if ((rc = D.dporder.alloc(sizeof(int32_t) * order.size()))) return rc;
  CKM_CUDA(cudaMemcpyAsync(D.dporder.p, order.data(), sizeof(int32_t) * order.size(), cudaMemcpyHostToDevice, st));
  p.pair_order = D.dporder.as<int32_t>();
  if ((rc = launch_class_runs(e, order, pcls, 0, (size_t)npairs, [&](int c, int32_t b0, int32_t b1, int grid, cudaStream_t s) -> int {
        p.pair_begin = b0; p.pair_end = b1; return c < N_BLK_CLASSES ? launch_regions2(p, c, grid, s) : launch_regions(p, grid, s); }))) return rc;
  if ((rc = fan_in(e))) return rc;
  int32_t nreg = 0;
  CKM_CUDA(cudaMemcpyAsync(&nreg, e->d_counters + CTR_ENV, sizeof(int32_t), cudaMemcpyDeviceToHost, st));
  CKM_CUDA(cudaStreamSynchronize(st));
  tr.mark("regions kernels");
  if (nreg > region_cap) { set_error("region queue overflow"); return CKM_ECAPACITY; }
  D.regs.resize((size_t)nreg);
  if (nreg) CKM_CUDA(cudaMemcpy(D.regs.data(), D.dregions.p, sizeof(Region) * D.regs.size(), cudaMemcpyDeviceToHost));
  std::sort(D.regs.begin(), D.regs.end(), [](const Region &a, const Region &b) { return a.pair != b.pair ? a.pair < b.pair : a.i < b.i; });
  tr.mark("regions sorted");
  return CKM_OK;
}

struct AbandonJob { cudaStream_t st; void operator()(EnsembleJob *job) const { ensembles_abandon(job, st); } };
static int domain_pass(ckm_engine *e, const SearchKnobs &k, const ckm_models *m, std::vector<PairWork> &pairs, DomainStage &D,
                       const std::vector<int> &multi_idx, std::vector<EnsembleCaps> &caps, Trace &tr, bool *grown) {
  cudaStream_t st = e->stream;
  DomdefParams &p = D.p;
  const std::vector<Region> &regs = D.regs; const int nreg = (int)regs.size();
  int rc;
  *grown = false;
  std::vector<int32_t> reg_slot((size_t)nreg);
  std::vector<Envelope> envs1, envs2;
  int32_t nslots = 0;
  for (auto &pw : pairs) { pw.ndom_slots = 0; pw.first_dom = 0; }
  for (int r = 0, mi = 0; r < nreg; ++r) {
    PairWork &pw = pairs[regs[r].pair];
    if (pw.ndom_slots == 0) pw.first_dom = nslots;
    reg_slot[r] = nslots;
    if (!regs[r].multi) { Envelope en{}; en.pair = regs[r].pair; en.i = regs[r].i; en.j = regs[r].j; en.slot = nslots; envs1.push_back(en); }
    const int n = regs[r].multi ? caps[mi++].envelopes : 1;
    nslots += n; pw.ndom_slots += n;
  }
  D.doms.assign((size_t)nslots, DomainOut{});
  if (nslots == 0) return CKM_OK;
  if ((rc = D.ddoms.alloc(sizeof(DomainOut) * (size_t)nslots)) || (rc = D.dhits.alloc(sizeof(HitOut) * pairs.size()))) return rc;
  CKM_CUDA(cudaMemsetAsync(D.ddoms.p, 0, sizeof(DomainOut) * (size_t)nslots, st));
  CKM_CUDA(cudaMemcpyAsync(D.dpairs.p, pairs.data(), sizeof(PairWork) * pairs.size(), cudaMemcpyHostToDevice, st));
  p.doms = D.ddoms.as<DomainOut>();
  const bool multi = !multi_idx.empty();
  bool ens_first = (k.ens_first == 1);
  if (k.ens_first < 0 && multi) {
    int64_t tot = 0;
    for (const Envelope &en : envs1) tot += envelope_need(m, pairs[en.pair], en, p.use_blk != 0);
    ens_first = tot > k.env_budget;
  }
  std::unique_ptr<EnsembleJob, AbandonJob> ens(nullptr, AbandonJob{e->aux});
  auto launch_ensemble = [&]() -> int {
    CKM_CUDA(cudaEventRecord(e->fan_ev, st));
    CKM_CUDA(cudaStreamWaitEvent(e->aux, e->fan_ev, 0));
    EnsembleJob *job = nullptr;
    const int r = ensembles_launch(e, m, p, pairs, regs, multi_idx, caps, e->aux, &job);
    ens.reset(job);
    return r;
  };
  if (multi && ens_first && (rc = launch_ensemble())) return rc;
  if ((rc = run_envelope_waves(e, m, pairs, p, k.env_budget, D.dscratch, envs1, D.denvs, D.deorder, multi))) return rc;
  tr.mark("envelope batch 1 launched");
  if (multi) {
    if (!ens_first && (rc = launch_ensemble())) return rc;
    if (!envs1.empty()) { if ((rc = fan_in(e))) return rc; CKM_CUDA(cudaStreamSynchronize(st)); }
    std::vector<std::vector<Envelope>> multi_envs; std::vector<EnsembleCaps> grow;
    int n_over = 0;
    if ((rc = ensembles_collect(ens.release(), e->aux, multi_envs, grow, &n_over))) return rc;
    tr.mark("batch 1 + ensemble done");
    if (n_over > 0) {
      for (size_t mi = 0; mi < caps.size(); ++mi) if (grow[mi].segments) caps[mi] = grow[mi];
      *grown = true;
      return CKM_OK;
    }
    for (size_t mi = 0; mi < multi_idx.size(); ++mi) {
      int c = 0;
      for (Envelope en : multi_envs[mi]) { en.slot = reg_slot[multi_idx[mi]] + c++; envs2.push_back(en); }
    }
    if ((rc = run_envelope_waves(e, m, pairs, p, k.env_budget, D.dscratch, envs2, D.denvs2, D.deorder2, false))) return rc;
    tr.mark("envelope batch 2 done");
  }
  p.hits = D.dhits.as<HitOut>();
  if ((rc = launch_scores(p, ((int)pairs.size() + 127) / 128, st))) return rc;
  e->stats.kernel_launches++;
  CKM_CUDA(cudaMemcpyAsync(D.doms.data(), D.ddoms.p, sizeof(DomainOut) * D.doms.size(), cudaMemcpyDeviceToHost, st));
  CKM_CUDA(cudaMemcpyAsync(D.hout.data(), D.dhits.p, sizeof(HitOut) * D.hout.size(), cudaMemcpyDeviceToHost, st));
  CKM_CUDA(cudaStreamSynchronize(st));
  return CKM_OK;
}
constexpr int DOMAIN_PASSES = 4;
static int run_domain_phase(ckm_engine *e, const SearchKnobs &k, const ckm_models *m, std::vector<PairWork> &pairs, DomainStage &D, Trace &tr) {
  std::vector<int> multi_idx;
  for (int r = 0; r < (int)D.regs.size(); ++r) if (D.regs[r].multi) multi_idx.push_back(r);
  std::vector<EnsembleCaps> caps(multi_idx.size(), ENS_DEFAULT_CAPS);
  D.hout.assign(pairs.size(), HitOut{});
  for (int pass = 0; pass < DOMAIN_PASSES; ++pass) {
    if (pass > 0) e->stats.n_queue_retries++;
    bool grown = false;
    int rc = domain_pass(e, k, m, pairs, D, multi_idx, caps, tr, &grown);
    if (rc || !grown) return rc;
  }
  set_error("a multi-domain region keeps outgrowing the capacities it asked for");
  return CKM_ECAPACITY;
}

static std::vector<ckm_hit> assemble_rows(ckm_engine *e, const ckm_models *m, const ckm_seqdb *db, const QueryPlan &q, const std::vector<PairWork> &pairs,
                                          const std::vector<HitOut> &hout, const std::vector<DomainOut> &doms, double Ecut, double domEcut) {
  struct Key { int bin, q, pair; double lnP; int seq; };
  std::vector<Key> keys;
  for (int i = 0; i < (int)pairs.size(); ++i) {
    if (!hout[i].valid) continue;
    const int b = db->bin_of_seq[pairs[i].seq];
    keys.push_back(Key{b, (q.per_bin ? q.qorder[b] : q.qorder[0])[pairs[i].model], i, hout[i].lnP, pairs[i].seq});
  }
  std::sort(keys.begin(), keys.end(), [](const Key &a, const Key &b) {
    if (a.bin != b.bin) return a.bin < b.bin;
    if (a.q != b.q) return a.q < b.q;
    if (a.lnP != b.lnP) return a.lnP < b.lnP;
    return a.seq < b.seq;
  });
  std::vector<ckm_hit> rows_out;
  size_t g0 = 0;
  int64_t n_dom = 0;
  for (size_t i = 0; i < doms.size(); ++i) if (doms[i].ok) n_dom++;
  while (g0 < keys.size()) {
    size_t g1 = g0;
    while (g1 < keys.size() && keys[g1].bin == keys[g0].bin && keys[g1].q == keys[g0].q) ++g1;
    const double Z = (double)db->bin_nseq[keys[g0].bin];
    double domZ = 0.0;
    for (size_t k = g0; k < g1; ++k) if (std::exp(keys[k].lnP) * Z <= Ecut) domZ += 1.0;
    for (size_t k = g0; k < g1; ++k) {
      if (!(std::exp(keys[k].lnP) * Z <= Ecut)) continue;
      const PairWork &pw = pairs[keys[k].pair];
      const HitOut &h = hout[keys[k].pair];
      int nrep = 0;
      for (int d = pw.first_dom; d < pw.first_dom + pw.ndom_slots; ++d)
        if (doms[d].ok && std::exp(doms[d].lnP) * domZ <= domEcut) nrep++;
      int nd = 0;
      for (int d = pw.first_dom; d < pw.first_dom + pw.ndom_slots; ++d) {
        const DomainOut &dm = doms[d];
        if (!dm.ok || !(std::exp(dm.lnP) * domZ <= domEcut)) continue;
        ckm_hit r;
        std::memset(&r, 0, sizeof(r));
        r.bin = keys[k].bin; r.seq = pw.seq; r.model = pw.model; r.tlen = pw.L; r.qlen = m->models[pw.model].M;
        r.dom = ++nd; r.ndom = nrep;
        r.hmm_from = dm.hmmfrom; r.hmm_to = dm.hmmto; r.ali_from = dm.sqfrom; r.ali_to = dm.sqto; r.env_from = dm.ienv; r.env_to = dm.jenv;
        r.full_score = h.score; r.full_bias = h.pre_score - h.score;
        r.dom_score = dm.bitscore; r.dom_bias = (float)((double)dm.dombias * 1.44269504088896341);
        r.acc = (float)(dm.oasc / (1.0 + std::fabs((float)(dm.jenv - dm.ienv))));
        r.full_evalue = std::exp(h.lnP) * Z; r.c_evalue = std::exp(dm.lnP) * domZ; r.i_evalue = std::exp(dm.lnP) * Z;
        r.full_lnP = h.lnP; r.dom_lnP = dm.lnP;
        rows_out.push_back(r);
      }
    }
    g0 = g1;
  }
  e->stats.n_hits_seq = (int64_t)keys.size(); e->stats.n_domains = n_dom; e->stats.n_reported = (int64_t)rows_out.size();
  return rows_out;
}

static int do_search(ckm_engine *e, const SearchKnobs &k, const ckm_models *m, const int32_t *model_idx, int32_t nmodels,
                     const int64_t *bin_model_offsets, const ckm_seqdb *db, double Ecut, double domEcut, ckm_hit **hits_out, int64_t *nhits_out) {
  cudaStream_t st = e->stream;
  *hits_out = nullptr; *nhits_out = 0;
  PoolScope pool_scope(e);
  QueryPlan q;
  int rc = plan_queries(m, db, model_idx, nmodels, bin_model_offsets, q, st);
  if (rc) return rc;
  std::memset(&e->stats, 0, sizeof(e->stats));
  if (q.n_pairs > ((int64_t)1 << 40)) { set_error("ckm_search: more than 2^40 (ORF x HMM) pairs in one call; search fewer bins per call"); return CKM_ECAPACITY; }
  CKM_CUDA(cudaEventRecord(e->ev[EV_CALL], st));
  Trace tr(k.trace);
  Stage1 s1; Stage2 s2; int32_t ctr[CTR_N];
  if ((rc = run_cascade(e, k, m, db, q.am, q.n_pairs, s1, s2, ctr))) return rc;
  tr.mark("filters done");
  std::vector<PairWork> pairs; int64_t rows = 0;
  if ((rc = sorted_pairs(db, s2.a.as<Candidate>(), ctr[CTR_FWD], pairs, rows))) return rc;
  CKM_CUDA(cudaEventRecord(e->ev[EV_DOMDEF], st));
  tr.mark("pair list sorted");
  DomainStage D;
  if (!pairs.empty()) {
    if ((rc = run_regions(e, k, m, db, pairs, rows, D, tr))) return rc;
    if ((rc = run_domain_phase(e, k, m, pairs, D, tr))) return rc;
  }
  CKM_CUDA(cudaEventRecord(e->ev[EV_END], st));
  CKM_CUDA(cudaEventSynchronize(e->ev[EV_END]));
  tr.mark("scores + downloads");
  const std::vector<ckm_hit> rows_out = assemble_rows(e, m, db, q, pairs, D.hout, D.doms, Ecut, domEcut);
  tr.mark("rows assembled");
  cudaEventElapsedTime(&e->stats.ms_domdef, e->ev[EV_DOMDEF], e->ev[EV_END]);
  cudaEventElapsedTime(&e->stats.ms_total, e->ev[EV_CALL], e->ev[EV_END]);
  if (!rows_out.empty()) {
    ckm_hit *out = (ckm_hit *)std::malloc(sizeof(ckm_hit) * rows_out.size());
    if (!out) { set_error("out of host memory"); return CKM_ENOMEM; }
    std::memcpy(out, rows_out.data(), sizeof(ckm_hit) * rows_out.size());
    *hits_out = out;
  }
  *nhits_out = (int64_t)rows_out.size();
  return CKM_OK;
}

static int align_pass(ckm_engine *e, const SearchKnobs &k, const ckm_models *m, const ckm_seqdb *db, std::vector<PairWork> &pairs,
                      std::vector<Envelope> &envs, int64_t rows, std::vector<int32_t> &trace, std::vector<DomainOut> &doms) {
  cudaStream_t st = e->stream;
  PoolScope pool_scope(e);
  DevBuf dpairs, dn2, dtrace, ddoms, dscratch, denvs, deorder;
  int rc;
  const size_t rws = (size_t)rows;
  if ((rc = dpairs.alloc(sizeof(PairWork) * pairs.size())) || (rc = dn2.alloc(sizeof(float) * rws)) || (rc = dtrace.alloc(sizeof(int32_t) * rws)) ||
      (rc = ddoms.alloc(sizeof(DomainOut) * pairs.size()))) return rc;
  CKM_CUDA(cudaMemcpyAsync(dpairs.p, pairs.data(), sizeof(PairWork) * pairs.size(), cudaMemcpyHostToDevice, st));
  CKM_CUDA(cudaMemsetAsync(dn2.p, 0, sizeof(float) * rws, st));
  CKM_CUDA(cudaMemsetAsync(dtrace.p, 0, sizeof(int32_t) * rws, st));
  CKM_CUDA(cudaMemsetAsync(ddoms.p, 0, sizeof(DomainOut) * pairs.size(), st));
  DomdefParams p = domdef_params(m, db, k);
  p.pairs = dpairs.as<PairWork>(); p.npairs = (int32_t)pairs.size();
  p.n2sc = dn2.as<float>(); p.trace = dtrace.as<int32_t>();
  p.doms = ddoms.as<DomainOut>();
  if ((rc = run_envelope_waves(e, m, pairs, p, k.env_budget, dscratch, envs, denvs, deorder, false))) return rc;
  trace.resize(rws);
  doms.resize(pairs.size());
  CKM_CUDA(cudaMemcpyAsync(trace.data(), dtrace.p, sizeof(int32_t) * rws, cudaMemcpyDeviceToHost, st));
  CKM_CUDA(cudaMemcpyAsync(doms.data(), ddoms.p, sizeof(DomainOut) * doms.size(), cudaMemcpyDeviceToHost, st));
  CKM_CUDA(cudaStreamSynchronize(st));
  return CKM_OK;
}

static int do_align(ckm_engine *e, const SearchKnobs &k, const ckm_models *m, int32_t model, const ckm_seqdb *db, int32_t *state_out, float *oasc_out) {
  std::memset(&e->stats, 0, sizeof(e->stats));
  const int nseq = db->nseq;
  for (int64_t i = 0; i < db->nres; ++i) state_out[i] = 0;
  if (oasc_out) for (int s = 0; s < nseq; ++s) oasc_out[s] = 0.0f;
  std::vector<PairWork> pairs;
  std::vector<Envelope> envs;
  int64_t rows = 0;
  auto add = [&](int s, int i, int j) {
    PairWork pw{};
    pw.seq = s; pw.model = model; pw.L = db->len[s]; pw.first_dom = (int32_t)pairs.size(); pw.ndom_slots = 1; pw.row_off = rows;
    rows += pw.L + 1;
    Envelope en{};
    en.pair = (int32_t)pairs.size(); en.i = i; en.j = j; en.null2_done = 1; en.slot = (int32_t)pairs.size();
    pairs.push_back(pw); envs.push_back(en);
  };
  for (int s = 0; s < nseq; ++s) if (db->len[s] > 0) add(s, 1, db->len[s]);
  if (pairs.empty()) return CKM_OK;
  std::vector<int32_t> trace; std::vector<DomainOut> doms;
  int rc;
  if ((rc = align_pass(e, k, m, db, pairs, envs, rows, trace, doms))) return rc;
  auto emit = [&](const std::vector<PairWork> &pp, const std::vector<DomainOut> &dd, const std::vector<int32_t> &tr, std::vector<int> *failed) {
    for (size_t pi = 0; pi < pp.size(); ++pi) {
      const PairWork &pw = pp[pi];
      if (!dd[pi].ok) { if (failed) failed->push_back(pw.seq); continue; }
      if (oasc_out) oasc_out[pw.seq] = dd[pi].oasc;
      int32_t *dst = state_out + (db->offsets[pw.seq] - db->offsets[0]);
      for (int i = 1; i <= pw.L; ++i) dst[i - 1] = tr[pw.row_off + i];
    }
  };
  std::vector<int> failed;
  emit(pairs, doms, trace, &failed);
  if (failed.empty()) return CKM_OK;
  ckm_hit *hits = nullptr; int64_t nhits = 0;
  if ((rc = do_search(e, k, m, &model, 1, nullptr, db, 1e300, 1e300, &hits, &nhits))) return rc;
  std::vector<int> best(nseq, -1);
  for (int64_t h = 0; h < nhits; ++h) { const int s = hits[h].seq; if (best[s] < 0 || hits[h].dom_score > hits[best[s]].dom_score) best[s] = (int)h; }
  pairs.clear(); envs.clear(); rows = 0;
  for (int s : failed) if (best[s] >= 0) add(s, hits[best[s]].env_from, hits[best[s]].env_to);
  std::free(hits);
  if (pairs.empty()) return CKM_OK;
  if ((rc = align_pass(e, k, m, db, pairs, envs, rows, trace, doms))) return rc;
  emit(pairs, doms, trace, nullptr);
  return CKM_OK;
}

static int checked_search(ckm_engine *e, const ckm_models *m, const int32_t *model_idx, int32_t nmodels, const int64_t *bin_model_offsets,
                          const ckm_seqdb *db, double E, double domE, ckm_hit **hits_out, int64_t *nhits_out) {
  if (!e || !m || !db || !hits_out || !nhits_out) { set_error("ckm_search: bad argument"); return CKM_EINVAL; }
  cudaSetDevice(e->device);
  return do_search(e, read_knobs(true), m, model_idx, nmodels, bin_model_offsets, db, E, domE, hits_out, nhits_out);
}

}

extern "C" {

int ckm_search(ckm_engine *e, const ckm_models *m, const int32_t *model_idx, int32_t nmodels,
               const ckm_seqdb *db, double E, double domE, ckm_hit **hits_out, int64_t *nhits_out) {
  return checked_search(e, m, model_idx, nmodels, nullptr, db, E, domE, hits_out, nhits_out);
}
int ckm_search_per_bin(ckm_engine *e, const ckm_models *m, const int32_t *model_idx, const int64_t *bin_model_offsets,
                       const ckm_seqdb *db, double E, double domE, ckm_hit **hits_out, int64_t *nhits_out) {
  if (!model_idx || !bin_model_offsets) { set_error("ckm_search_per_bin: bad argument"); return CKM_EINVAL; }
  return checked_search(e, m, model_idx, 0, bin_model_offsets, db, E, domE, hits_out, nhits_out);
}
int ckm_align(ckm_engine *e, const ckm_models *m, int32_t model, const ckm_seqdb *db, int32_t *state_out, float *oasc_out) {
  if (!e || !m || !db || !state_out) { set_error("ckm_align: bad argument"); return CKM_EINVAL; }
  if (model < 0 || model >= (int)m->models.size()) { set_error("ckm_align: model index out of range"); return CKM_EINVAL; }
  cudaSetDevice(e->device);
  return do_align(e, read_knobs(true), m, model, db, state_out, oasc_out);
}

int ckm_write_domtblout(const ckm_models *m, const ckm_hit *hits, int64_t nhits, int32_t bin, int32_t seq_base,
                        const char *const *names, const char *const *descs, const char *path) {
  if (!m || (!hits && nhits > 0) || !names || !path) { set_error("ckm_write_domtblout: bad argument"); return CKM_EINVAL; }
  FILE *fp = std::fopen(path, "w");
  if (!fp) { set_error(std::string("cannot write ") + path); return CKM_EIO; }
  int tnamew = 20, qnamew = 20, qaccw = 10, taccw = 10;
  for (int64_t i = 0; i < nhits; ++i) {
    if (hits[i].bin != bin) continue;
    const Model &md = m->models[hits[i].model];
    tnamew = std::max<int>(tnamew, (int)std::strlen(names[hits[i].seq - seq_base]));
    qnamew = std::max<int>(qnamew, (int)md.name.size());
    qaccw = std::max<int>(qaccw, (int)md.acc.size());
  }
  std::fprintf(fp, "#%*s %22s %40s %11s %11s %11s\n", tnamew + qnamew - 1 + 15 + taccw + qaccw, "", "--- full sequence ---",
               "-------------- this domain -------------", "hmm coord", "ali coord", "env coord");
  std::fprintf(fp, "#%-*s %-*s %5s %-*s %-*s %5s %9s %6s %5s %3s %3s %9s %9s %6s %5s %5s %5s %5s %5s %5s %5s %4s %s\n",
               tnamew - 1, " target name", taccw, "accession", "tlen", qnamew, "query name", qaccw, "accession", "qlen",
               "E-value", "score", "bias", "#", "of", "c-Evalue", "i-Evalue", "score", "bias", "from", "to", "from", "to", "from", "to", "acc", "description of target");
  std::fprintf(fp, "#%*s %*s ----- %*s %*s ----- --------- ------ ----- --- --- --------- --------- ------ ----- ----- ----- ----- ----- ----- ----- ---- ---------------------\n",
               tnamew - 1, "-------------------", taccw, "----------", qnamew, "--------------------", qaccw, "----------");
  for (int64_t i = 0; i < nhits; ++i) {
    const ckm_hit &h = hits[i];
    if (h.bin != bin) continue;
    const Model &md = m->models[h.model];
    const char *desc = (descs && descs[h.seq - seq_base] && descs[h.seq - seq_base][0]) ? descs[h.seq - seq_base] : "-";
    std::fprintf(fp, "%-*s %-*s %5d %-*s %-*s %5d %9.2g %6.1f %5.1f %3d %3d %9.2g %9.2g %6.1f %5.1f %5d %5d %5d %5d %5d %5d %4.2f %s\n",
                 tnamew, names[h.seq - seq_base], taccw, "-", h.tlen, qnamew, md.name.c_str(), qaccw, md.acc.empty() ? "-" : md.acc.c_str(), h.qlen,
                 h.full_evalue, h.full_score, h.full_bias, h.dom, h.ndom, h.c_evalue, h.i_evalue, h.dom_score, h.dom_bias,
                 h.hmm_from, h.hmm_to, h.ali_from, h.ali_to, h.env_from, h.env_to, h.acc, desc);
  }
  std::fprintf(fp, "#\n# Program:         checkm_b200 (libckm.so)\n# Pipeline mode:   SEARCH\n# [ok]\n");
  std::fclose(fp);
  return CKM_OK;
}

int ckm_filter_scores(ckm_engine *e, const ckm_models *m, const int32_t *model_idx, int32_t nmodels,
                      const ckm_seqdb *db, float *filtersc_out, float *vit_out, float *fwd_out, uint8_t *passed_out) {
  if (!e || !m || !db || !filtersc_out || !vit_out || !fwd_out || !passed_out) { set_error("ckm_filter_scores: bad argument"); return CKM_EINVAL; }
  cudaSetDevice(e->device);
  const SearchKnobs k = read_knobs(false);
  PoolScope pool_scope(e);
  QueryPlan q;
  int rc = plan_queries(m, db, model_idx, nmodels, nullptr, q, e->stream);
  if (rc) return rc;
  const int64_t n = q.n_pairs;
  DevBuf dfs, dvit, dfwd, dpass;
  const size_t nf = (size_t)std::max<int64_t>(n, 1);
  if ((rc = dfs.alloc(sizeof(float) * nf)) || (rc = dvit.alloc(sizeof(float) * nf)) || (rc = dfwd.alloc(sizeof(float) * nf)) ||
      (rc = dpass.alloc(nf + 4))) return rc;
  for (DevBuf *b : {&dfs, &dvit, &dfwd}) CKM_CUDA(cudaMemsetAsync(b->p, 0xff, sizeof(float) * nf, e->stream));
  CKM_CUDA(cudaMemsetAsync(dpass.p, 0, nf + 4, e->stream));
  Stage1 s1; Stage2 s2;
  std::memset(&e->stats, 0, sizeof(e->stats));
  if ((rc = run_stage1(e, k, m, db, q.am, n, s1, nullptr))) return rc;
  if ((rc = run_stage2(e, k, m, db, q.am, s1, s2, dfs.as<float>(), dvit.as<float>(), dfwd.as<float>(), dpass.as<uint8_t>()))) return rc;
  int32_t ctr[CTR_N];
  CKM_CUDA(cudaMemcpyAsync(ctr, e->d_counters, sizeof(ctr), cudaMemcpyDeviceToHost, e->stream));
  CKM_CUDA(cudaMemcpyAsync(filtersc_out, dfs.p, sizeof(float) * (size_t)n, cudaMemcpyDeviceToHost, e->stream));
  CKM_CUDA(cudaMemcpyAsync(vit_out, dvit.p, sizeof(float) * (size_t)n, cudaMemcpyDeviceToHost, e->stream));
  CKM_CUDA(cudaMemcpyAsync(fwd_out, dfwd.p, sizeof(float) * (size_t)n, cudaMemcpyDeviceToHost, e->stream));
  CKM_CUDA(cudaMemcpyAsync(passed_out, dpass.p, (size_t)n, cudaMemcpyDeviceToHost, e->stream));
  CKM_CUDA(cudaStreamSynchronize(e->stream));
  if (ctr[CTR_CAND] > s1.cand_cap || ctr[CTR_MSV] > s1.pass_cap) { set_error("candidate queue overflow"); return CKM_ECAPACITY; }
  std::vector<Candidate> pass1((size_t)ctr[CTR_MSV]);
  if (!pass1.empty()) CKM_CUDA(cudaMemcpy(pass1.data(), s1.pass.p, sizeof(Candidate) * pass1.size(), cudaMemcpyDeviceToHost));
  for (const Candidate &c : pass1) passed_out[(int64_t)q.qorder[0][c.model] * db->nseq + c.seq] |= 1;
  fill_filter_stats(e, n, ctr,  0, 5);
  return CKM_OK;
}

int ckm_viterbi_scores(ckm_engine *e, const ckm_models *m, const int32_t *model_idx, int32_t nmodels,
                       const ckm_seqdb *db, int32_t mode, float *vit_out) {
  if (!e || !m || !db || !vit_out) { set_error("ckm_viterbi_scores: bad argument"); return CKM_EINVAL; }
  cudaSetDevice(e->device);
  cudaStream_t st = e->stream;
  const int ndb = (int)m->models.size();
  if (model_idx == nullptr) nmodels = ndb;
  const int64_t n = (int64_t)nmodels * db->nseq;
  if (n > ((int64_t)1 << 30)) { set_error("ckm_viterbi_scores: too many pairs for one call"); return CKM_ECAPACITY; }
  PoolScope pool_scope(e);
  ActiveMasks am; std::vector<int32_t> slot;
  int rc = build_masks(m, db, model_idx, nmodels, nullptr, am, slot, st);
  if (rc) return rc;
  std::vector<int32_t> slot_model((size_t)std::max(nmodels, 1));
  for (int i = 0; i < nmodels; ++i) slot_model[i] = model_idx ? model_idx[i] : i;
  const size_t nf = (size_t)std::max<int64_t>(n, 1);
  DevBuf dsm, din, dout, dredo, dvit, dgrp;
  if ((rc = dsm.alloc(sizeof(int32_t) * slot_model.size())) || (rc = din.alloc(sizeof(Candidate) * nf)) || (rc = dout.alloc(sizeof(Candidate) * nf)) ||
      (rc = dredo.alloc(sizeof(Candidate) * nf)) || (rc = dvit.alloc(sizeof(float) * nf))) return rc;
  CKM_CUDA(cudaMemcpyAsync(dsm.p, slot_model.data(), sizeof(int32_t) * slot_model.size(), cudaMemcpyHostToDevice, st));
  CKM_CUDA(cudaMemsetAsync(e->d_counters, 0, CTR_N * sizeof(int32_t), st));
  CKM_CUDA(cudaMemsetAsync(dvit.p, 0xff, sizeof(float) * nf, st));
  std::memset(&e->stats, 0, sizeof(e->stats));
  if (n > 0) {
    if ((rc = launch_all_pairs(din.as<Candidate>(), e->d_counters + CTR_BIAS, dsm.as<int32_t>(), nmodels, db->nseq, st))) return rc;
    FilterParams p = filter_params(m, db, am);
    p.use_blk = (mode == 2) ? 0 : 1;
    p.dense_vit = dvit.as<float>();
    p.redo = dredo.as<Candidate>(); p.redo_count = e->d_counters + CTR_VREDO; p.redo_cap = (int32_t)nf;
    p.in = din.as<Candidate>(); p.in_count = e->d_counters + CTR_BIAS; p.in_cap = (int32_t)nf;
    p.out = dout.as<Candidate>(); p.out_count = e->d_counters + CTR_VIT; p.out_cap = (int32_t)nf;
    if ((rc = run_viterbi(e, m, p, mode == 0, dgrp))) return rc;
  }
  int32_t ctr[CTR_N];
  CKM_CUDA(cudaMemcpyAsync(ctr, e->d_counters, sizeof(ctr), cudaMemcpyDeviceToHost, st));
  CKM_CUDA(cudaMemcpyAsync(vit_out, dvit.p, sizeof(float) * (size_t)n, cudaMemcpyDeviceToHost, st));
  CKM_CUDA(cudaStreamSynchronize(st));
  e->stats.n_pairs = n; e->stats.n_past_bias = ctr[CTR_BIAS]; e->stats.n_past_vit = ctr[CTR_VIT]; e->stats.n_vit_redo = ctr[CTR_VREDO];
  return CKM_OK;
}

int ckm_msv_scores(ckm_engine *e, const ckm_models *m, const int32_t *model_idx, int32_t nmodels,
                   const ckm_seqdb *db, int32_t *xj_out) {
  if (!e || !m || !db || !xj_out) { set_error("ckm_msv_scores: bad argument"); return CKM_EINVAL; }
  cudaSetDevice(e->device);
  const SearchKnobs k = read_knobs(false);
  PoolScope pool_scope(e);
  QueryPlan q;
  int rc = plan_queries(m, db, model_idx, nmodels, nullptr, q, e->stream);
  if (rc) return rc;
  const int64_t n = q.n_pairs;
  DevBuf dense;
  if ((rc = dense.alloc(sizeof(int32_t) * (size_t)std::max<int64_t>(n, 1)))) return rc;
  CKM_CUDA(cudaMemsetAsync(dense.p, 0xff, sizeof(int32_t) * (size_t)n, e->stream));
  Stage1 s1;
  std::memset(&e->stats, 0, sizeof(e->stats));
  if ((rc = run_stage1(e, k, m, db, q.am, n, s1, dense.as<int32_t>()))) return rc;
  int32_t ctr[CTR_N];
  CKM_CUDA(cudaMemcpyAsync(ctr, e->d_counters, sizeof(ctr), cudaMemcpyDeviceToHost, e->stream));
  unsigned long long cells = 0;
  CKM_CUDA(cudaMemcpyAsync(&cells, s1.cells.p, sizeof(cells), cudaMemcpyDeviceToHost, e->stream));
  CKM_CUDA(cudaMemcpyAsync(xj_out, dense.p, sizeof(int32_t) * (size_t)n, cudaMemcpyDeviceToHost, e->stream));
  CKM_CUDA(cudaStreamSynchronize(e->stream));
  if (ctr[CTR_CAND] > s1.cand_cap || ctr[CTR_MSV] > s1.pass_cap) { set_error("candidate queue overflow"); return CKM_ECAPACITY; }
  fill_filter_stats(e, n, ctr, cells, 2);
  return CKM_OK;
}

}
```

### checkm_b200/csrc/stages.hpp

```cpp
#pragma once
#include <type_traits>
#include "engine.hpp"

namespace ckm {

#ifndef CKM_SSV_WARPS
#define CKM_SSV_WARPS 16
#endif
constexpr int SSV_WARPS = CKM_SSV_WARPS;
constexpr int SSV_WARPS_HOST = SSV_WARPS;
constexpr int MSV_WARPS = 8;

struct SsvParams {
  const uint8_t *res; const int64_t *off; const int32_t *len; const int32_t *bin;
  const float *msvB; const int32_t *tjb; const int32_t *order;
  int32_t nseq, seq_chunk, nchunks;
  const TileGroup *groups; const int32_t *group_list; int32_t ngroups;
  const TileDesc *tiles; const TileModel *tile_models;
  const int32_t *chain_first_tile, *chain_ntiles;
  const uint8_t *tile_blob;
  const uint8_t *tile_active;
  const uint8_t *model_active;
  int32_t ntiles, nmodels;
  int32_t *unit_counter;
  int2 *cand; int32_t *cand_count; int32_t cand_cap;
  int16_t *bnd; int64_t bnd_stride;
  unsigned long long *cells;
  int32_t resolve;
  const ModelScalars *ms; const float *nullsc;
  Candidate *pass; int32_t *pass_count; int32_t pass_cap;
  int32_t *resolved_count;
  int32_t *xj_dense; const int32_t *model_slot;
  double F1;
};

int launch_ssv(int J, const SsvParams &p, int grid, size_t smem_bytes, cudaStream_t stream);

struct MsvParams {
  const uint8_t *res; const int64_t *off; const int32_t *len;
  const float *nullsc; const int32_t *tjb;
  const ModelScalars *ms; const uint8_t *rbv; const uint32_t *rmb;
  const int2 *cand; const int32_t *cand_count; int32_t cand_cap;
  Candidate *out; int32_t *out_count; int32_t out_cap;
  int32_t *xj_dense;
  const int32_t *model_slot;
  int32_t nseq;
  int32_t row_bytes;
  int32_t use_blk;
  double F1;
};

int launch_msv_exact(const MsvParams &p, int grid, cudaStream_t stream);
int launch_ssv_bypass(const int32_t *models, int32_t nbypass, int32_t nseq, const int32_t *len, const int32_t *bin,
                      const uint8_t *model_active, int32_t nmodels_db, int2 *cand, int32_t *cand_count, int32_t cand_cap,
                      cudaStream_t stream);
int launch_msv2(const MsvParams &p, int cls, int grid, cudaStream_t stream);

constexpr int VIT_WARPS = 4;
constexpr int FWD_WARPS = 4;
struct FilterParams {
  const uint8_t *res; const int64_t *off; const int32_t *len;
  const float *lenA, *lenB;
  const int16_t *tmove_w;
  const ModelScalars *ms;
  const float *bias_eo; const int16_t *rwv; const int16_t *twv; const float *rfv; const float *tfv;
  const uint4 *twb; const uint32_t *rwb; const float4 *tfb; const float *rfb;
  const uint4 *twp; const uint32_t *rwp;
  Candidate *redo; int32_t *redo_count; int32_t redo_cap;
  int32_t *vit_idx; int2 *vit_chunks; int32_t *vit_cls_chunks; int32_t *vit_work;
  const Candidate *in; const int32_t *in_count; int32_t in_cap;
  Candidate *out; int32_t *out_count; int32_t out_cap;
  int32_t row_elems;
  double F1, F2, F3;
  int32_t use_blk;
  float *dense_filtersc, *dense_vit, *dense_fwd; uint8_t *dense_passed;
  const int32_t *model_slot; int32_t nseq;
};
int launch_bias(const FilterParams &p, int grid, cudaStream_t st);
int launch_vit(const FilterParams &p, int grid, cudaStream_t st);
constexpr int N_BLK_CLASSES = 10;
constexpr int BLK_Q[N_BLK_CLASSES] = {2, 4, 6, 8, 12, 16, 20, 24, 28, 32};
constexpr bool blk_tsmem(int q) { return q >= 12; }
__host__ __device__ constexpr int vq_of(int M) { return M <= 256 ? 2 * ((M + 63) / 64) : M <= 1024 ? 4 * ((M + 127) / 128) : 0; }
__host__ __device__ constexpr int blk_class(int vq) { return vq == 0 ? N_BLK_CLASSES : (vq <= 8 ? vq / 2 - 1 : vq / 4 + 1); }
constexpr bool blk_table_ok(int c = 0) {
  return c == N_BLK_CLASSES || (blk_class(BLK_Q[c]) == c && vq_of(32 * BLK_Q[c]) == BLK_Q[c] &&
                                vq_of(32 * BLK_Q[c] + 1) == (c + 1 < N_BLK_CLASSES ? BLK_Q[c + 1] : 0) && blk_table_ok(c + 1));
}
static_assert(vq_of(1) == 2 && blk_table_ok(), "lane-block class arithmetic disagrees with BLK_Q");

template <int C = 0, class F> int with_class(int cls, F &&f) {
  if constexpr (C == N_BLK_CLASSES) {
    set_error("bad lane-block class " + std::to_string(cls));
    return CKM_EINVAL;
  } else {
    if (cls == C) return f(std::integral_constant<int, BLK_Q[C]>{}, std::integral_constant<bool, blk_tsmem(BLK_Q[C])>{});
    return with_class<C + 1>(cls, f);
  }
}

template <class... KA, class... A>
int launch_kernel(void (*kern)(KA...), const char *name, int grid, int block, size_t smem, cudaStream_t st, const A &...args) {
  cudaError_t e;
  if (smem > 48 * 1024 && (e = cudaFuncSetAttribute(kern, cudaFuncAttributeMaxDynamicSharedMemorySize, (int)smem)) != cudaSuccess)
    return cuda_fail(e, name);
  kern<<<grid, block, smem, st>>>(args...);
  e = cudaGetLastError();
  return e == cudaSuccess ? CKM_OK : cuda_fail(e, name);
}

int launch_vit2(const FilterParams &p, int cls, int grid, cudaStream_t st);
int launch_vitp(const FilterParams &p, int cls, int grid, cudaStream_t st);
constexpr int VITP_CHUNK = 64;
int launch_vit_group(const FilterParams &p, int32_t nmodels, int32_t *ws, int grid, cudaStream_t st);
int launch_all_pairs(Candidate *out, int32_t *count, const int32_t *slot_model, int32_t nslots, int32_t nseq, cudaStream_t st);
int launch_fwd(const FilterParams &p, int grid, cudaStream_t st);

#define FLT_MIN_F 1.17549435e-38f
struct PairWork {
  int32_t seq, model, L;
  int32_t first_dom, ndom_slots;
  float   fwdsc, filtersc, usc;
  int64_t row_off;
};
struct Region { int32_t pair, i, j, multi; };
constexpr int ENS_MAXENV = 32;
struct EnsembleCaps { int32_t segments, trace_segments, envelopes; };
constexpr EnsembleCaps ENS_DEFAULT_CAPS = {4096, 64, ENS_MAXENV};
struct Envelope { int32_t pair, i, j, null2_done; int64_t scratch_off; int32_t slot, pad; };
struct DomainOut {
  int32_t pair, ienv, jenv, hmmfrom, hmmto, sqfrom, sqto, ok;
  float   envsc, domcorrection, oasc, bitscore, dombias, pad;
  double  lnP;
};
struct HitOut { float pre_score, score, sum_score; int32_t ndom, valid, pad; double lnP; };
struct DomdefParams {
  const uint8_t *res; const int64_t *off; const float *nullsc;
  const ModelScalars *ms; const float *rfv; const float *tfv;
  const PairWork *pairs; int32_t npairs;
  const int32_t *pair_order; int32_t pair_begin, pair_end;
  float *xf, *xb, *btot, *etot, *mocc, *n2sc;
  int32_t *trace;
  Region *regions; int32_t *region_count; int32_t region_cap;
  const Envelope *envs; const int32_t *env_order; int32_t env_begin, env_end;
  float *scratch;
  DomainOut *doms; HitOut *hits;
  const float *logsum_tbl;
  int32_t row_elems;
  const float4 *tfb; const float *rfb;
  int32_t use_blk;
};
int launch_regions(const DomdefParams &p, int grid, cudaStream_t st);
int launch_envelopes(const DomdefParams &p, int grid, cudaStream_t st);
int launch_scores(const DomdefParams &p, int grid, cudaStream_t st);
int launch_fwd2(const FilterParams &p, int cls, int grid, cudaStream_t st);
int launch_regions2(const DomdefParams &p, int cls, int grid, cudaStream_t st);
int launch_envelopes2(const DomdefParams &p, int cls, int grid, cudaStream_t st);

}
```

### include/ckm.h

```cpp
#ifndef CKM_H
#define CKM_H
#include <stdint.h>

#ifdef __cplusplus
extern "C" {
#endif

typedef enum {
  CKM_OK = 0,
  CKM_EINVAL = 1,
  CKM_EIO = 2,
  CKM_EFORMAT = 3,
  CKM_ENODEVICE = 4,
  CKM_ECUDA = 5,
  CKM_ENOMEM = 6,
  CKM_ENOTFOUND = 7,
  CKM_ECAPACITY = 8
} ckm_status;

typedef struct ckm_engine   ckm_engine;
typedef struct ckm_models   ckm_models;
typedef struct ckm_seqdb    ckm_seqdb;

typedef struct {
  char   name[128];
  char   acc[64];
  char   desc[256];
  int32_t M;
  int32_t has_ga, has_tc, has_nc;
  float  ga[2], tc[2], nc[2];
  float  evparam[6];
  double ga_d[2], tc_d[2], nc_d[2];
} ckm_model_info;

typedef struct {
  int32_t bin;
  int32_t seq;
  int32_t model;
  int32_t tlen;
  int32_t qlen;
  int32_t dom, ndom;
  int32_t hmm_from, hmm_to, ali_from, ali_to, env_from, env_to;
  float   full_score, full_bias;
  float   dom_score, dom_bias;
  float   acc;
  double  full_evalue, c_evalue, i_evalue;
  double  full_lnP, dom_lnP;
} ckm_hit;

typedef struct {
  int64_t n_pairs;
  int64_t n_cells;
  int64_t n_ssv_cand;
  int64_t n_past_msv, n_past_bias, n_past_vit, n_past_fwd;
  int64_t n_hits_seq;
  int64_t n_domains;
  int64_t n_reported;
  float   ms_ssv, ms_msv, ms_bias, ms_vit, ms_fwd, ms_domdef, ms_total;
  int64_t kernel_launches;
  int64_t n_vit_redo;
  int64_t n_msv_exact;
  int64_t n_queue_retries;
} ckm_stats;

typedef struct {
  int32_t bin;
  int32_t counts[6];
  int32_t n_markers, n_sets;
  int32_t unique_hits, multi_hits;
  double  completeness, contamination;
} ckm_qa_row;

typedef struct {
  int32_t bin, model;
  int32_t seq_a, seq_b;
  int32_t target_length;
  int32_t hmm_from, hmm_to, ali_from, ali_to, env_from, env_to;
  int32_t order;
  int32_t src_row;
  int64_t dict_key;
} ckm_marker_hit;

int  ckm_init(int device, ckm_engine **out);
void ckm_destroy(ckm_engine *e);
const char *ckm_last_error(void);
const char *ckm_version(void);
int  ckm_device_name(ckm_engine *e, char *buf, int buflen);

int  ckm_models_load(ckm_engine *e, const char *hmm_path, ckm_models **out);
int  ckm_models_count(const ckm_models *m);
int  ckm_models_info(const ckm_models *m, int idx, ckm_model_info *out);
int  ckm_models_find(const ckm_models *m, const char *key);
int  ckm_models_select(const ckm_models *m, const char *const *keys, int nkeys, int32_t *idx_out, int *n_out);
int  ckm_models_write(const ckm_models *m, const int32_t *idx, int n, const char *out_path);
void ckm_models_free(ckm_models *m);

int  ckm_digitize(const char *text, int64_t n, uint8_t *out);
int  ckm_fasta_parse(const char *text, int64_t n, uint8_t *residues_out, int64_t *offsets_out, int32_t max_records,
                     char *headers_out, int64_t headers_cap, int32_t *nrec_out, int64_t *nres_out, int64_t *hdr_bytes_out);
int  ckm_seqdb_create(ckm_engine *e, const uint8_t *residues, const int64_t *seq_offsets, int32_t nseq,
                      const int32_t *bin_of_seq, int32_t nbins, ckm_seqdb **out);
void ckm_seqdb_free(ckm_seqdb *db);

int  ckm_search(ckm_engine *e, const ckm_models *m, const int32_t *model_idx, int32_t nmodels,
                const ckm_seqdb *db, double E, double domE, ckm_hit **hits_out, int64_t *nhits_out);
int  ckm_search_per_bin(ckm_engine *e, const ckm_models *m, const int32_t *model_idx, const int64_t *bin_model_offsets,
                        const ckm_seqdb *db, double E, double domE, ckm_hit **hits_out, int64_t *nhits_out);
void ckm_hits_free(ckm_hit *hits);

int  ckm_align(ckm_engine *e, const ckm_models *m, int32_t model, const ckm_seqdb *db, int32_t *state_out, float *oasc_out);
int  ckm_last_stats(const ckm_engine *e, ckm_stats *out);

int  ckm_msv_scores(ckm_engine *e, const ckm_models *m, const int32_t *model_idx, int32_t nmodels,
                    const ckm_seqdb *db, int32_t *xj_out );
int  ckm_filter_scores(ckm_engine *e, const ckm_models *m, const int32_t *model_idx, int32_t nmodels,
                       const ckm_seqdb *db, float *filtersc_out, float *vit_out, float *fwd_out,
                       uint8_t *passed_out );

int  ckm_viterbi_scores(ckm_engine *e, const ckm_models *m, const int32_t *model_idx, int32_t nmodels,
                        const ckm_seqdb *db, int32_t mode, float *vit_out );

int  ckm_write_domtblout(const ckm_models *m, const ckm_hit *hits, int64_t nhits, int32_t bin,
                         int32_t seq_base, const char *const *names, const char *const *descs, const char *path);

typedef struct {
  int32_t ignore_thresholds;
  int32_t skip_pseudogene;
  int32_t skip_adjacent;
  int32_t individual_markers;
  double  evalue_threshold;
  int32_t evalue_exp10;
  int32_t pad0;
  double  evalue_mant;
  double  length_threshold;
  double  pseudogene_length;
} ckm_reduce_opts;

typedef struct {
  const uint8_t *is_pfam, *is_tigr;
  const int32_t *clan;
  const int64_t *nest_off; const int32_t *nest_idx;
  const int32_t *has_cut;
  const double  *cutoffs;
  const double  *row_scores;
  const int32_t *scaffold_id, *orf_num;
  const int32_t *name_rank;
  const int64_t *bin_set_off;
  const int64_t *set_marker_off;
  const int32_t *set_marker_idx;
} ckm_reduce_meta;

int  ckm_reduce(ckm_engine *e, int32_t nmodels, int32_t nseq, int32_t nbins, const ckm_hit *hits, int64_t nhits,
                const ckm_reduce_opts *opts, const ckm_reduce_meta *meta,
                ckm_qa_row **qa_out, int32_t *nqa_out, ckm_marker_hit **mh_out, int64_t *nmh_out);
int  ckm_genome_check(ckm_engine *e, int32_t nbins, const int64_t *bin_set_off, const int64_t *set_marker_off,
                      const int32_t *marker_count, int32_t individual_markers, ckm_qa_row *rows_out);
void ckm_free(void *p);

int  ckm_nccl_unique_id(uint8_t *id_out, int32_t nbytes);
int  ckm_nccl_comm_init(ckm_engine *e, int32_t world, int32_t rank, const uint8_t *id, void **comm_out);
void ckm_nccl_comm_destroy(void *comm);
int  ckm_allgather_qa(ckm_engine *e, void *nccl_comm, const ckm_qa_row *rows, int32_t nrows, int32_t nrows_max,
                      int32_t world, ckm_qa_row *rows_out, int32_t *counts_out);

int  ckm_fasta_scan_nt(const char *text, int64_t n, uint8_t *bytes_out, int64_t bytes_cap, int64_t *starts_out, int64_t *lens_out,
                       int32_t max_records, char *headers_out, int64_t headers_cap, int32_t *nrec_out, int64_t *bytes_used_out,
                       int64_t *hdr_bytes_out);
int  ckm_scaffold_stats(ckm_engine *e, const uint8_t *bytes, int64_t nbytes, const int64_t *starts, const int64_t *lens,
                        int32_t nscaf, int64_t *stats_out, uint32_t *contig_scaffold_out, uint32_t *contig_len_out,
                        int64_t contig_cap, int64_t *ncontigs_out, float *kernel_ms_out);

int  ckm_kmer_counts(ckm_engine *e, const uint8_t *bytes, int64_t nbytes, const int64_t *starts, const int64_t *lens,
                     int32_t nseq, int32_t k, uint32_t *counts_out, float *kernel_ms_out);
int  ckm_kmer_columns(int32_t k, char *out);
int  ckm_format_kmer_profiles(const uint32_t *counts, int32_t nseq, int32_t k, const char *ids, const int64_t *id_offsets,
                              char *out, int64_t out_cap, int64_t *out_len);

typedef struct { int32_t i, j, p, s; } ckm_merge_pair;
int  ckm_merge_pairs(ckm_engine *e, const int32_t *counts, int32_t nbins, int32_t nmarkers, const int32_t *n_markers,
                     double min_delta_comp, double max_delta_cont, double min_merged_comp, double max_merged_cont,
                     ckm_merge_pair *pairs_out, int64_t pair_cap, int64_t *npairs_out, float *kernel_ms_out);
int  ckm_format_merger_rows(const char *ids, const int64_t *id_offsets, int32_t nbins, const int32_t *p, const int32_t *s,
                            const int32_t *n_markers, const ckm_merge_pair *pairs, int64_t npairs, char *out, int64_t out_cap,
                            int64_t *out_len);

int  ckm_parse_kmer_profiles(const char *text, int64_t n, int32_t ncols, int32_t nthreads, int64_t *id_start_out,
                             int32_t *id_len_out, double *values_out, int64_t row_cap, int64_t *nrows_out);
typedef struct ckm_sigs ckm_sigs;
int  ckm_sigs_create(ckm_engine *e, const double *values, int64_t nrows, ckm_sigs **out);
void ckm_sigs_free(ckm_sigs *s);
typedef struct {
  int64_t nseq;
  int32_t nbins, ntables;
  const int64_t *bin_off;
  const int64_t *len;
  const int64_t *acgt;
  const int64_t *coding;
  const int64_t *sig_row;
  const int32_t *bin_gc_table;
  const int32_t *bin_cd_table;
  int32_t td_table, pad;
  const int64_t *table_off;
  const double *table_key;
  const double *table_lo;
  const double *table_hi;
  const double *binsig_in;
} ckm_outlier_in;
typedef struct {
  double *bin_means;
  double *bin_sig;
  double *seq_values;
  uint8_t *seq_mask;
  float kernel_ms[3];
} ckm_outlier_out;
int  ckm_outlier_scores(ckm_engine *e, const ckm_sigs *sigs, const ckm_outlier_in *in, ckm_outlier_out *out);

typedef struct { int64_t coffset; int32_t clen; int32_t isize; } ckm_bgzf_block;
int  ckm_bgzf_blocks(const uint8_t *data, int64_t n, int64_t base, ckm_bgzf_block *blocks_out, int64_t cap,
                     int64_t *nblocks_out, int64_t *consumed_out);
int  ckm_bgzf_inflate(ckm_engine *e, const uint8_t *comp, int64_t comp_base, int64_t comp_len, const ckm_bgzf_block *blocks,
                      int64_t nblocks, uint8_t *out, int64_t out_cap, int64_t *bad_block_out, float *kernel_ms_out);
typedef struct {
  int32_t all_reads;
  int32_t min_qc;
  double  min_align;
  double  max_edit;
} ckm_bam_filter;
int  ckm_bam_coverage(ckm_engine *e, const uint8_t *comp, int64_t comp_base, int64_t comp_len, const ckm_bgzf_block *blocks,
                      int64_t nblocks, const int64_t *seg_start, const int64_t *seg_end, int64_t nseg, int32_t n_ref,
                      const ckm_bam_filter *filter, int64_t *counters, float *kernel_ms_out, int64_t *err_offset_out);
int  ckm_bam_windows(ckm_engine *e, const uint8_t *comp, int64_t comp_base, int64_t comp_len, const ckm_bgzf_block *blocks,
                     int64_t nblocks, const int64_t *seg_start, const int64_t *seg_end, int64_t nseg, int32_t n_ref,
                     const ckm_bam_filter *filter, const int64_t *ref_len, int64_t window_size, const int64_t *win_off,
                     int64_t *counters, int64_t *windows, float *kernel_ms_out, int64_t *err_offset_out);

int  ckm_window_stats(ckm_engine *e, const uint8_t *bytes, int64_t nbytes, const int64_t *starts, const int64_t *lens,
                      int32_t nseq, int64_t window_size, const int64_t *win_off, const double *bin_sig, int64_t *acgt_out,
                      double *td_out, float *kernel_ms_out);

int  ckm_id_join(ckm_engine *e, const char *text, int64_t nbytes, int32_t nbins, const int64_t *bin_nrec, int64_t nasm,
                 int64_t *id_start_out, int64_t *id_len_out, uint8_t *asm_flags_out, int32_t *asm_last_out,
                 uint8_t *bin_keep_out, int64_t *n_binned_ids_out, int64_t *bad_record_out, float *kernel_ms_out);
int  ckm_format_unbinned(const char *ids, const int64_t *id_start, const int64_t *id_len, const uint8_t *bytes,
                         const int64_t *starts, const int64_t *lens, const int64_t *acgt, int64_t n, char *fasta_out,
                         int64_t fasta_cap, char *stats_out, int64_t stats_cap, int64_t *fasta_len_out, int64_t *stats_len_out);

#ifdef __cplusplus
}
#endif
#endif
```

Before: 35480.

## Group forward and large-envelope work by model with block-shared model tables

Forward-filter candidates, and envelope jobs for large model classes, are grouped by model into chunks using the count/scan/scatter machinery previously built for Viterbi. Each block claims a chunk through an atomic cursor and loads that model's transition table, plus the emission table for small Q, into shared memory once. All warps then process that model's sequences from shared memory, replacing per-warp global loads of the model. This adds extra grouping kernels, host-side sorting by model and larger shared-memory footprints, which may reduce occupancy. It also adds envelope and region counters to the stats.

Measured after the change: 36050, median of 6. 1.6% higher.

```diff
diff --git a/checkm_b200/_lib.py b/checkm_b200/_lib.py
--- a/checkm_b200/_lib.py
+++ b/checkm_b200/_lib.py
@@ -30,7 +30,8 @@
                 ("ms_ssv", C.c_float), ("ms_msv", C.c_float), ("ms_bias", C.c_float), ("ms_vit", C.c_float),
                 ("ms_fwd", C.c_float), ("ms_domdef", C.c_float), ("ms_total", C.c_float),
                 ("kernel_launches", C.c_int64), ("n_vit_redo", C.c_int64), ("n_msv_exact", C.c_int64),
-                ("n_queue_retries", C.c_int64)]
+                ("n_queue_retries", C.c_int64), ("n_regions", C.c_int64), ("n_multi_regions", C.c_int64),
+                ("n_envelopes", C.c_int64), ("n_env_waves", C.c_int64)]
 
 
 class QaRow(C.Structure):
diff --git a/checkm_b200/csrc/fwdback_blk.cuh b/checkm_b200/csrc/fwdback_blk.cuh
--- a/checkm_b200/csrc/fwdback_blk.cuh
+++ b/checkm_b200/csrc/fwdback_blk.cuh
@@ -7,8 +7,9 @@
 
 constexpr int BLK_LOOKAHEAD_MAXQ = 16;
 
-template <int Q, bool TSMEM>
+template <int Q_, bool TSMEM, bool ESMEM>
 struct BlkModel {
+  static constexpr int Q = Q_;
   int M;
   const float *rfb;
   const float4 *tsm;
@@ -16,10 +17,11 @@
   int lane;
   __device__ __forceinline__ float4 T0(int q) const { return TSMEM ? tsm[q * 32 + lane] : t0[TSMEM ? 0 : q]; }
   __device__ __forceinline__ float4 T1(int q) const { return TSMEM ? tsm[(Q + q) * 32 + lane] : t1[TSMEM ? 0 : q]; }
+  __device__ __forceinline__ float E(const float *rp, int q) const { return ESMEM ? rp[q * 32] : __ldg(rp + q * 32); }
 };
 
 template <int Q, bool TSMEM>
-__device__ __forceinline__ void blk_model_load(BlkModel<Q, TSMEM> &bm, const ModelScalars &ms, const float4 *tfb, const float *rfb,
+__device__ __forceinline__ void blk_model_load(BlkModel<Q, TSMEM, false> &bm, const ModelScalars &ms, const float4 *tfb, const float *rfb,
                                                float4 *tsm, int lane) {
   bm.M = ms.M; bm.lane = lane;
   bm.rfb = rfb + ms.blk_off * 32 * KPAD + lane;
@@ -35,8 +37,8 @@
   }
 }
 
-template <int Q, bool TSMEM, bool FULL, bool STORE_D = true>
-__device__ __forceinline__ float forward_blk(const BlkModel<Q, TSMEM> &bm, const uint8_t *__restrict__ res, int L, const Specials sp,
+template <bool FULL, bool STORE_D = true, int Q, bool TSMEM, bool ESMEM>
+__device__ __forceinline__ float forward_blk(const BlkModel<Q, TSMEM, ESMEM> &bm, const uint8_t *__restrict__ res, int L, const Specials sp,
                                              float *xmx, float *full) {
   const int lane = bm.lane;
   float Mx[Q], Ix[Q], Dx[Q];
@@ -54,7 +56,7 @@
   if (LA) {
     const float *rp = bm.rfb + (size_t)((L >= 1) ? __ldg(res) : 0) * Q * 32;
 #pragma unroll
-    for (int q = 0; q < Q; ++q) ecur[q] = __ldg(rp + q * 32);
+    for (int q = 0; q < Q; ++q) ecur[q] = bm.E(rp, q);
     xnext = (L >= 2) ? __ldg(res + 1) : 0;
   } else xnext = (L >= 1) ? __ldg(res) : 0;
   for (int i = 1; i <= L; ++i) {
@@ -63,11 +65,11 @@
       const float *rp = bm.rfb + (size_t)xnext * Q * 32;
       if (LA) {
 #pragma unroll
-        for (int q = 0; q < Q; ++q) enext[LA ? q : 0] = __ldg(rp + q * 32);
+        for (int q = 0; q < Q; ++q) enext[LA ? q : 0] = bm.E(rp, q);
         xnext = (i + 2 <= L) ? __ldg(res + i + 1) : 0;
       } else {
 #pragma unroll
-        for (int q = 0; q < Q; ++q) ecur[q] = __ldg(rp + q * 32);
+        for (int q = 0; q < Q; ++q) ecur[q] = bm.E(rp, q);
         xnext = (i + 1 <= L) ? __ldg(res + i) : 0;
       }
     }
@@ -139,8 +141,8 @@
 }
 
 __device__ __forceinline__ void prefetch_l2(const void *p) { asm volatile("prefetch.global.L2 [%0];" ::"l"(p)); }
-template <int Q, bool TSMEM, int MODE>
-__device__ __forceinline__ void backward_blk(const BlkModel<Q, TSMEM> &bm, const uint8_t *__restrict__ res, int L, const Specials sp,
+template <int MODE, int Q, bool TSMEM, bool ESMEM>
+__device__ __forceinline__ void backward_blk(const BlkModel<Q, TSMEM, ESMEM> &bm, const uint8_t *__restrict__ res, int L, const Specials sp,
                                              const float *fxmx, float *bxmx, float *full) {
   const int lane = bm.lane, M = bm.M;
   float Mx[Q], Ix[Q], Dx[Q];
@@ -157,12 +159,12 @@
     if (LA) {
       const float *rp = bm.rfb + (size_t)xnext * Q * 32;
 #pragma unroll
-      for (int q = 0; q < Q; ++q) enext[LA ? q : 0] = __ldg(rp + q * 32);
+      for (int q = 0; q < Q; ++q) enext[LA ? q : 0] = bm.E(rp, q);
       xnext = (i >= 2) ? __ldg(res + i - 2) : 0;
     } else if (i < L) {
       const float *rp = bm.rfb + (size_t)xnext * Q * 32;
 #pragma unroll
-      for (int q = 0; q < Q; ++q) ecur[q] = __ldg(rp + q * 32);
+      for (int q = 0; q < Q; ++q) ecur[q] = bm.E(rp, q);
       xnext = (i >= 1) ? __ldg(res + i - 1) : 0;
     }
     if (MODE == 2 && i >= 3) {
diff --git a/checkm_b200/csrc/kernels_blk.cu b/checkm_b200/csrc/kernels_blk.cu
--- a/checkm_b200/csrc/kernels_blk.cu
+++ b/checkm_b200/csrc/kernels_blk.cu
@@ -12,22 +12,69 @@
 
 __host__ __device__ constexpr size_t blk_tsm_bytes(int Q) { return (size_t)Q * 32 * 2 * sizeof(float4); }
 
+__host__ __device__ constexpr bool blk_esmem(int Q) { return Q <= 20; }
+__host__ __device__ constexpr size_t blk_grouped_smem_bytes(int Q) { return blk_tsm_bytes(Q) + (blk_esmem(Q) ? (size_t)KPAD * Q * 32 * sizeof(float) : 0); }
+
+template <int Q, bool TSMEM, class ModelOf, class Body>
+__device__ __forceinline__ void blk_chunks(const int2 *chunks, int nch, int32_t *cursor, const ModelScalars *msv, const float4 *tfb,
+                                           const float *rfb, ModelOf model_of, Body body) {
+  constexpr bool ESMEM = blk_esmem(Q);
+  extern __shared__ __align__(16) uint8_t bsm[];
+  __shared__ int s_chunk, s_next, s_end;
+  __shared__ ModelScalars s_ms;
+  float4 *tsm = reinterpret_cast<float4 *>(bsm);
+  float *esm = reinterpret_cast<float *>(bsm + blk_tsm_bytes(Q));
+  const int lane = threadIdx.x & 31;
+  for (;;) {
+    __syncthreads();
+    if (threadIdx.x == 0) {
+      const int k = atomicAdd(cursor, 1);
+      s_chunk = k;
+      if (k < nch) { s_next = chunks[k].x; s_end = chunks[k].y; s_ms = msv[model_of(s_next)]; }
+    }
+    __syncthreads();
+    const int k = s_chunk;
+    if (k >= nch) break;
+    const ModelScalars &ms = s_ms;
+    {
+      const float4 *tsrc = tfb + ms.blk_off * 32 * 2;
+      for (int z = threadIdx.x; z < Q * 64; z += blockDim.x) tsm[(z & 1) * (Q * 32) + (z >> 1)] = __ldg(tsrc + z);
+      if (ESMEM) {
+        const float4 *esrc = reinterpret_cast<const float4 *>(rfb + ms.blk_off * 32 * KPAD);
+        float4 *edst = reinterpret_cast<float4 *>(esm);
+        for (int z = threadIdx.x; z < KPAD * Q * 8; z += blockDim.x) edst[z] = __ldg(esrc + z);
+      }
+    }
+    __syncthreads();
+    for (;;) {
+      int j = 0;
+      if (lane == 0) j = atomicAdd(&s_next, 1);
+      j = __shfl_sync(0xffffffffu, j, 0);
+      if (j >= s_end) break;
+      BlkModel<Q, TSMEM, ESMEM> bm;
+      bm.M = ms.M; bm.lane = lane; bm.tsm = tsm;
+      bm.rfb = (ESMEM ? esm : rfb + ms.blk_off * 32 * KPAD) + lane;
+      if (!TSMEM) {
+#pragma unroll
+        for (int q = 0; q < Q; ++q) { bm.t0[TSMEM ? 0 : q] = tsm[q * 32 + lane]; bm.t1[TSMEM ? 0 : q] = tsm[(Q + q) * 32 + lane]; }
+      }
+      body(bm, ms, j);
+      __syncwarp();
+    }
+  }
+}
+
 template <int Q, bool TSMEM>
-__global__ void __launch_bounds__(BLK_WARPS * 32) fwd2_kernel(FilterParams p) {
-  extern __shared__ __align__(16) uint8_t bsm[];
-  const int lane = threadIdx.x & 31, warp = threadIdx.x >> 5;
-  float4 *tsm = reinterpret_cast<float4 *>(bsm) + (size_t)warp * Q * 32 * 2;
-  const int n = min(*p.in_count, p.in_cap);
-  for (int c = blockIdx.x * BLK_WARPS + warp; c < n; c += gridDim.x * BLK_WARPS) {
-    Candidate cd = p.in[c];
-    const ModelScalars ms = p.ms[cd.model];
-    if (ms.vq != Q) continue;
-    const int s = cd.seq, L = p.len[s];
-    BlkModel<Q, TSMEM> bm;
-    blk_model_load<Q, TSMEM>(bm, ms, p.tfb, p.rfb, tsm, lane);
-    const float fsc = forward_blk<Q, TSMEM, false>(bm, p.res + p.off[s], L, make_specials(L, true), nullptr, nullptr);
-    fwd_verdict(p, cd, fsc, ms, lane);
-  }
+__global__ void __launch_bounds__(BLK_WARPS * 32) fwd2_kernel(FilterParams p, int cls) {
+  const int c0 = p.grp_cls_chunks[cls];
+  blk_chunks<Q, TSMEM>(p.grp_chunks + c0, p.grp_cls_chunks[cls + 1] - c0, p.grp_work + cls, p.ms, p.tfb, p.rfb,
+                       [&](int j) { return p.in[p.grp_idx[j]].model; },
+                       [&](const auto &bm, const ModelScalars &ms, int j) {
+                         Candidate cd = p.in[p.grp_idx[j]];
+                         const int s = cd.seq, L = p.len[s];
+                         const float fsc = forward_blk<false>(bm, p.res + p.off[s], L, make_specials(L, true), nullptr, nullptr);
+                         fwd_verdict(p, cd, fsc, ms, bm.lane);
+                       });
 }
 
 template <int Q, bool TSMEM>
@@ -41,14 +88,14 @@
     const ModelScalars ms = p.ms[pw.model];
     if (ms.vq != Q) continue;
     const int L = pw.L;
-    BlkModel<Q, TSMEM> bm;
+    BlkModel<Q, TSMEM, false> bm;
     blk_model_load<Q, TSMEM>(bm, ms, p.tfb, p.rfb, tsm, lane);
     const uint8_t *res = p.res + p.off[pw.seq];
     const Specials sp = make_specials(L, true);
     float *xf = p.xf + pw.row_off * X_NX, *xb = p.xb + pw.row_off * X_NX;
-    forward_blk<Q, TSMEM, false>(bm, res, L, sp, xf, nullptr);
-    __syncwarp();
-    backward_blk<Q, TSMEM, 0>(bm, res, L, sp, xf, xb, nullptr);
+    forward_blk<false>(bm, res, L, sp, xf, nullptr);
+    __syncwarp();
+    backward_blk<0>(bm, res, L, sp, xf, xb, nullptr);
     __syncwarp();
     regions_tail(p, pi, L, sp, xf, xb, p.btot + pw.row_off, p.etot + pw.row_off, p.mocc + pw.row_off, p.n2sc + pw.row_off, lane);
     __syncwarp();
@@ -89,19 +136,13 @@
 
 template <int Q, bool TSMEM>
 __global__ void __launch_bounds__(BLK_WARPS * 32) envelope2_kernel(DomdefParams p) {
+  constexpr bool GROUPED = blk_env_grouped(Q);
   extern __shared__ __align__(16) uint8_t bsm[];
   const int lane = threadIdx.x & 31, warp = threadIdx.x >> 5;
-  float4 *tsm = reinterpret_cast<float4 *>(bsm) + (size_t)warp * Q * 32 * 2;
-  float *null2 = reinterpret_cast<float *>(bsm + (TSMEM ? BLK_WARPS * blk_tsm_bytes(Q) : 0)) + warp * 32;
+  float *null2 = reinterpret_cast<float *>(bsm + (GROUPED ? blk_grouped_smem_bytes(Q) : TSMEM ? BLK_WARPS * blk_tsm_bytes(Q) : 0)) + warp * 32;
   constexpr int QW = Q * 32;
-  for (int idx = p.env_begin + blockIdx.x * BLK_WARPS + warp; idx < p.env_end; idx += gridDim.x * BLK_WARPS) {
-    const int ei = p.env_order[idx];
-    const Envelope env = p.envs[ei];
+  auto one = [&](const auto &bm, const ModelScalars &ms, const Envelope env) {
     const PairWork pw = p.pairs[env.pair];
-    const ModelScalars ms = p.ms[pw.model];
-    if (ms.vq != Q) continue;
-    BlkModel<Q, TSMEM> bm;
-    blk_model_load<Q, TSMEM>(bm, ms, p.tfb, p.rfb, tsm, lane);
     const int M = ms.M, Ld = env.j - env.i + 1;
     const uint8_t *res = p.res + p.off[pw.seq] + (env.i - 1);
     const Specials sp = make_specials(pw.L, false);
@@ -110,9 +151,9 @@
     float *xf = F + mat, *xb = xf + (int64_t)(Ld + 1) * X_NX, *pps = xb + (int64_t)(Ld + 1) * X_NX;
     float *xo = xf;
     float *n2sc = p.n2sc + pw.row_off;
-    const float envsc = forward_blk<Q, TSMEM, true, false>(bm, res, Ld, sp, xf, F);
-    __syncwarp();
-    backward_blk<Q, TSMEM, 2>(bm, res, Ld, sp, xf, xb, F);
+    const float envsc = forward_blk<true, false>(bm, res, Ld, sp, xf, F);
+    __syncwarp();
+    backward_blk<2>(bm, res, Ld, sp, xf, xb, F);
     __syncwarp();
     const float scaleproduct = __fdiv_rn(1.0f, xb[X_N]);
     float em[Q], ein[Q];
@@ -146,7 +187,7 @@
         const float *rp = bm.rfb + (size_t)x * QW;
         float part = 0.0f;
 #pragma unroll
-        for (int q = 0; q < Q; ++q) { part += em[q] * __ldg(rp + q * 32); part += ein[q]; }
+        for (int q = 0; q < Q; ++q) { part += em[q] * bm.E(rp, q); part += ein[q]; }
         part = warp_sum_float(part);
         if (lane == 0) null2[x] = part + xfactor;
       }
@@ -228,7 +269,21 @@
     OaTrace tr;
     if (!range_err) tr = oa_traceback(BlockedLayout<Q>{Bm, p.tfb + ms.blk_off * 64, M}, p, pw, env, sp, xo, pps, Ld, M, lane);
     write_domain(p, env, n2sc, tr, envsc, oasc, lane);
-    __syncwarp();
+  };
+  if constexpr (GROUPED) {
+    blk_chunks<Q, TSMEM>(p.chunks, p.nchunks, p.chunk_cursor, p.ms, p.tfb, p.rfb, [&](int j) { return p.pairs[p.envs[p.env_order[j]].pair].model; },
+                         [&](const auto &bm, const ModelScalars &ms, int j) { one(bm, ms, p.envs[p.env_order[j]]); });
+  } else {
+    float4 *tsm = reinterpret_cast<float4 *>(bsm) + (size_t)warp * Q * 32 * 2;
+    for (int idx = p.env_begin + blockIdx.x * BLK_WARPS + warp; idx < p.env_end; idx += gridDim.x * BLK_WARPS) {
+      const Envelope env = p.envs[p.env_order[idx]];
+      const ModelScalars ms = p.ms[p.pairs[env.pair].model];
+      if (ms.vq != Q) continue;
+      BlkModel<Q, TSMEM, false> bm;
+      blk_model_load<Q, TSMEM>(bm, ms, p.tfb, p.rfb, tsm, lane);
+      one(bm, ms, env);
+      __syncwarp();
+    }
   }
 }
 
@@ -237,14 +292,19 @@
   return launch_kernel(kern, name, grid, BLK_WARPS * 32, (tsmem ? BLK_WARPS * blk_tsm_bytes(Q) : 0) + extra, st, p);
 }
 int launch_fwd2(const FilterParams &p, int cls, int grid, cudaStream_t st) {
-  return with_class(cls, [&](auto Q, auto TSMEM) { return launch_blk(fwd2_kernel<Q, TSMEM>, "fwd2_kernel", Q, TSMEM, p, grid, 0, st); });
+  return with_class(cls, [&](auto Q, auto TSMEM) {
+    return launch_kernel(fwd2_kernel<Q, TSMEM>, "fwd2_kernel", grid, BLK_WARPS * 32, blk_grouped_smem_bytes(Q), st, p, cls);
+  });
 }
 int launch_regions2(const DomdefParams &p, int cls, int grid, cudaStream_t st) {
   return with_class(cls, [&](auto Q, auto TSMEM) { return launch_blk(regions2_kernel<Q, TSMEM>, "regions2_kernel", Q, TSMEM, p, grid, 0, st); });
 }
 int launch_envelopes2(const DomdefParams &p, int cls, int grid, cudaStream_t st) {
   return with_class(cls, [&](auto Q, auto TSMEM) {
-    return launch_blk(envelope2_kernel<Q, TSMEM>, "envelope2_kernel", Q, TSMEM, p, grid, BLK_WARPS * 32 * sizeof(float), st);
+    const size_t null2 = BLK_WARPS * 32 * sizeof(float);
+    if (blk_env_grouped(Q))
+      return launch_kernel(envelope2_kernel<Q, TSMEM>, "envelope2_kernel", grid, BLK_WARPS * 32, blk_grouped_smem_bytes(Q) + null2, st, p);
+    return launch_blk(envelope2_kernel<Q, TSMEM>, "envelope2_kernel", Q, TSMEM, p, grid, null2, st);
   });
 }
 
diff --git a/checkm_b200/csrc/kernels_vitp.cu b/checkm_b200/csrc/kernels_vitp.cu
--- a/checkm_b200/csrc/kernels_vitp.cu
+++ b/checkm_b200/csrc/kernels_vitp.cu
@@ -12,25 +12,28 @@
 __device__ __forceinline__ int vp_lo(uint32_t w) { return (int)(int16_t)(w & 0xffffu); }
 __device__ __forceinline__ int vp_hi(uint32_t w) { return (int)w >> 16; }
 
-__global__ void vit_count_kernel(FilterParams p, int32_t *cnt) {
+__device__ __forceinline__ bool group_listed(const FilterParams &p, const Candidate &cd, bool viterbi) {
+  return (!viterbi || cd.P > p.F2) && p.ms[cd.model].vq != 0;
+}
+__global__ void group_count_kernel(FilterParams p, bool viterbi, int32_t *cnt) {
   const int n = min(*p.in_count, p.in_cap);
   for (int i = blockIdx.x * blockDim.x + threadIdx.x; i < n; i += gridDim.x * blockDim.x) {
     const Candidate cd = p.in[i];
-    if (!(cd.P > p.F2)) filter_pass(p, cd, 4);
-    else if (p.ms[cd.model].vq == 0) vit_redo(p, cd);
-    else atomicAdd(cnt + cd.model, 1);
-  }
-}
-
-__global__ void __launch_bounds__(1024) vit_scan_kernel(FilterParams p, int32_t nmodels, const int32_t *cnt, int32_t *off, int32_t *choff) {
+    if (group_listed(p, cd, viterbi)) atomicAdd(cnt + cd.model, 1);
+    else if (viterbi && !(cd.P > p.F2)) filter_pass(p, cd, 4);
+    else if (viterbi) vit_redo(p, cd);
+  }
+}
+
+__global__ void __launch_bounds__(1024) group_scan_kernel(FilterParams p, int32_t nmodels, const int32_t *cnt, int32_t *off, int32_t *choff) {
   __shared__ int ws[2][32];
   const int lane = threadIdx.x & 31, warp = threadIdx.x >> 5;
   int run_pairs = 0, run_chunks = 0;
   for (int c = 0; c < N_BLK_CLASSES; ++c) {
-    if (threadIdx.x == 0) p.vit_cls_chunks[c] = run_chunks;
+    if (threadIdx.x == 0) p.grp_cls_chunks[c] = run_chunks;
     for (int b = 0; b < nmodels; b += 1024) {
       const int m = b + threadIdx.x;
-      const int v = (m < nmodels && blk_class(p.ms[m].vq) == c) ? cnt[m] : 0, h = (v + VITP_CHUNK - 1) / VITP_CHUNK;
+      const int v = (m < nmodels && blk_class(p.ms[m].vq) == c) ? cnt[m] : 0, h = (v + GROUP_CHUNK - 1) / GROUP_CHUNK;
       int sv = v, sh = h;
 #pragma unroll
       for (int o = 1; o < 32; o <<= 1) {
@@ -57,29 +60,29 @@
       __syncthreads();
     }
   }
-  if (threadIdx.x == 0) p.vit_cls_chunks[N_BLK_CLASSES] = run_chunks;
-}
-
-__global__ void vit_scatter_kernel(FilterParams p, const int32_t *cnt, int32_t *fill, const int32_t *off, const int32_t *choff) {
+  if (threadIdx.x == 0) p.grp_cls_chunks[N_BLK_CLASSES] = run_chunks;
+}
+
+__global__ void group_scatter_kernel(FilterParams p, bool viterbi, const int32_t *cnt, int32_t *fill, const int32_t *off, const int32_t *choff) {
   const int n = min(*p.in_count, p.in_cap);
   for (int i = blockIdx.x * blockDim.x + threadIdx.x; i < n; i += gridDim.x * blockDim.x) {
+    if (!group_listed(p, p.in[i], viterbi)) continue;
     const int m = p.in[i].model;
-    if (!(p.in[i].P > p.F2) || p.ms[m].vq == 0) continue;
     const int r = atomicAdd(fill + m, 1), pos = off[m] + r;
-    p.vit_idx[pos] = i;
-    if (r % VITP_CHUNK == 0) p.vit_chunks[choff[m] + r / VITP_CHUNK] = make_int2(pos, off[m] + min(r + VITP_CHUNK, cnt[m]));
-  }
-}
-
-int launch_vit_group(const FilterParams &p, int32_t nmodels, int32_t *ws, int grid, cudaStream_t st) {
+    p.grp_idx[pos] = i;
+    if (r % GROUP_CHUNK == 0) p.grp_chunks[choff[m] + r / GROUP_CHUNK] = make_int2(pos, off[m] + min(r + GROUP_CHUNK, cnt[m]));
+  }
+}
+
+int launch_group(const FilterParams &p, int32_t nmodels, int32_t *ws, bool viterbi, int grid, cudaStream_t st) {
   int32_t *cnt = ws, *fill = ws + nmodels, *off = ws + 2 * (size_t)nmodels, *choff = ws + 3 * (size_t)nmodels;
   cudaError_t e = cudaMemsetAsync(ws, 0, sizeof(int32_t) * 2 * (size_t)nmodels, st);
-  if (e != cudaSuccess) return cuda_fail(e, "cudaMemsetAsync(vit groups)");
-  vit_count_kernel<<<grid, 256, 0, st>>>(p, cnt);
-  vit_scan_kernel<<<1, 1024, 0, st>>>(p, nmodels, cnt, off, choff);
-  vit_scatter_kernel<<<grid, 256, 0, st>>>(p, cnt, fill, off, choff);
+  if (e != cudaSuccess) return cuda_fail(e, "cudaMemsetAsync(work groups)");
+  group_count_kernel<<<grid, 256, 0, st>>>(p, viterbi, cnt);
+  group_scan_kernel<<<1, 1024, 0, st>>>(p, nmodels, cnt, off, choff);
+  group_scatter_kernel<<<grid, 256, 0, st>>>(p, viterbi, cnt, fill, off, choff);
   e = cudaGetLastError();
-  return e == cudaSuccess ? CKM_OK : cuda_fail(e, "vit grouping launch");
+  return e == cudaSuccess ? CKM_OK : cuda_fail(e, "work grouping launch");
 }
 
 constexpr int VITP_THREADS = 128;
@@ -96,21 +99,21 @@
   uint4 *tws = vsm + KPAD * W * 8;
   const int lane = threadIdx.x & 31;
   const uint32_t sel = (lane == 0) ? 0x1054u : 0x3210u;
-  const int c0 = p.vit_cls_chunks[cls], nch = p.vit_cls_chunks[cls + 1] - c0;
+  const int c0 = p.grp_cls_chunks[cls], nch = p.grp_cls_chunks[cls + 1] - c0;
   for (;;) {
     __syncthreads();
     if (threadIdx.x == 0) {
-      const int k = atomicAdd(p.vit_work + cls, 1);
+      const int k = atomicAdd(p.grp_work + cls, 1);
       s_chunk = k;
       if (k < nch) {
-        s_next = p.vit_chunks[c0 + k].x;
-        s_ms = p.ms[p.in[p.vit_idx[s_next]].model];
+        s_next = p.grp_chunks[c0 + k].x;
+        s_ms = p.ms[p.in[p.grp_idx[s_next]].model];
       }
     }
     __syncthreads();
     const int k = s_chunk;
     if (k >= nch) break;
-    const int2 ch = p.vit_chunks[c0 + k];
+    const int2 ch = p.grp_chunks[c0 + k];
     const ModelScalars &ms = s_ms;
     {
       const uint4 *esrc = reinterpret_cast<const uint4 *>(p.rwp + ms.blk_off * 32 * (KPAD / 2));
@@ -137,7 +140,7 @@
       if (lane == 0) j = atomicAdd(&s_next, 1);
       j = __shfl_sync(0xffffffffu, j, 0);
       if (j >= ch.y) break;
-      const Candidate *cin = p.in + p.vit_idx[j];
+      const Candidate *cin = p.in + p.grp_idx[j];
       const int s = cin->seq, L = p.len[s];
       bool redo = false;
       const int tmove = p.tmove_w[s];
diff --git a/checkm_b200/csrc/search.cu b/checkm_b200/csrc/search.cu
--- a/checkm_b200/csrc/search.cu
+++ b/checkm_b200/csrc/search.cu
@@ -25,7 +25,8 @@
                      cudaStream_t st, EnsembleJob **job_out);
 int ensembles_collect(EnsembleJob *job, cudaStream_t st, std::vector<std::vector<Envelope>> &out, std::vector<EnsembleCaps> &grow, int *n_over);
 void ensembles_abandon(EnsembleJob *job, cudaStream_t st);
-enum { CTR_UNIT4 = 0, CTR_UNIT8, CTR_UNIT16, CTR_UNIT32, CTR_CAND, CTR_MSV, CTR_BIAS, CTR_VIT, CTR_FWD, CTR_ENV, CTR_DOM, CTR_VREDO, CTR_SSVRES, CTR_VWORK = 16 , CTR_N = 32 };
+enum { CTR_UNIT4 = 0, CTR_UNIT8, CTR_UNIT16, CTR_UNIT32, CTR_CAND, CTR_MSV, CTR_BIAS, CTR_VIT, CTR_FWD, CTR_ENV, CTR_DOM, CTR_VREDO, CTR_SSVRES, CTR_VWORK = 16 ,
+       CTR_FWORK = 32 , CTR_N = 48 };
 enum { EV_SSV = 0, EV_MSV, EV_BIAS, EV_VIT, EV_FWD, EV_CASCADE_END, EV_DOMDEF, EV_END, EV_CALL };
 
 static int64_t env_scratch_budget() {
@@ -92,19 +93,43 @@
   }
   return fan_in(e);
 }
-template <class Launch> static int launch_class_runs(ckm_engine *e, const std::vector<int32_t> &order, const std::vector<int8_t> &cls, size_t b0, size_t b1, Launch launch) {
+struct RunChunks { const int2 *chunks; int32_t n; int32_t *cursor; };
+template <class Launch> static int launch_class_runs(ckm_engine *e, const std::vector<int32_t> &order, const std::vector<int8_t> &cls, size_t b0, size_t b1, Launch launch,
+                                                     bool (*grouped)(int c) = nullptr, const std::vector<int32_t> *model = nullptr,
+                                                     int32_t *d_chunks = nullptr, RunChunks *run_chunks = nullptr) {
   const int nsm = e->prop.multiProcessorCount;
-  int rc;
+  struct Run { size_t b0, b1; int c; size_t ch0, nch; };
+  std::vector<Run> runs;
+  std::vector<int32_t> hw;
+  for (size_t r0 = b0, r1; r0 < b1; r0 = r1) {
+    const int c = cls[order[r0]];
+    for (r1 = r0; r1 < b1 && cls[order[r1]] == c; ++r1) {}
+    Run run{r0, r1, c, hw.size() / 2, 0};
+    for (size_t i = r0, j; grouped != nullptr && grouped(c) && i < r1; i = j, ++run.nch) {
+      for (j = i + 1; j < r1 && j < i + GROUP_CHUNK && (*model)[order[j]] == (*model)[order[i]]; ++j) {}
+      hw.push_back((int32_t)i); hw.push_back((int32_t)j);
+    }
+    runs.push_back(run);
+  }
+  const size_t ncur = hw.size();
+  int rc;
+  if (ncur > 0) {
+    hw.resize(ncur + runs.size(), 0);
+    CKM_CUDA(cudaMemcpyAsync(d_chunks, hw.data(), sizeof(int32_t) * hw.size(), cudaMemcpyHostToDevice, e->stream));
+  }
   if ((rc = fan_out(e))) return rc;
-  while (b0 < b1) {
-    size_t r1 = b0; const int c = cls[order[b0]];
-    while (r1 < b1 && cls[order[r1]] == c) ++r1;
-    const int cnt = (int)(r1 - b0);
-    const int grid = c < N_BLK_CLASSES ? std::min(nsm * 8, (cnt + 3) / 4) : std::min(nsm * 4, (cnt + FWD_WARPS - 1) / FWD_WARPS);
-    if ((rc = launch(c, (int32_t)b0, (int32_t)r1, grid, e->cls[c]))) return rc;
+  for (size_t r = 0; r < runs.size(); ++r) {
+    const Run &run = runs[r];
+    const int cnt = (int)(run.b1 - run.b0), c = run.c;
+    int grid = c < N_BLK_CLASSES ? std::min(nsm * 8, (cnt + 3) / 4) : std::min(nsm * 4, (cnt + FWD_WARPS - 1) / FWD_WARPS);
+    if (run.nch > 0) {
+      grid = std::min<int>(nsm * 8, (int)run.nch);
+      *run_chunks = RunChunks{reinterpret_cast<const int2 *>(d_chunks) + run.ch0, (int32_t)run.nch, d_chunks + ncur + r};
+    }
+    if ((rc = launch(c, (int32_t)run.b0, (int32_t)run.b1, grid, e->cls[c]))) return rc;
     e->stats.kernel_launches++;
-    b0 = r1;
-  }
+  }
+  if (ncur > 0) CKM_CUDA(cudaStreamSynchronize(e->stream));
   return CKM_OK;
 }
 
@@ -280,19 +305,23 @@
   return CKM_OK;
 }
 
+static int group_pairs(ckm_engine *e, const ckm_models *m, FilterParams &p, bool viterbi, int32_t *cursors, DevBuf &grp) {
+  const int nm = (int)m->models.size();
+  const size_t nchunks = (size_t)p.in_cap / GROUP_CHUNK + nm + 1;
+  const size_t words = 4 * (size_t)nm + 16 + ((size_t)p.in_cap + 1) / 2 * 2;
+  int rc;
+  if ((rc = grp.alloc(sizeof(int32_t) * words + sizeof(int2) * nchunks))) return rc;
+  int32_t *ws = grp.as<int32_t>();
+  p.grp_cls_chunks = ws + 4 * (size_t)nm;
+  p.grp_idx = p.grp_cls_chunks + 16;
+  p.grp_chunks = reinterpret_cast<int2 *>(ws + words);
+  p.grp_work = cursors;
+  return launch_group(p, nm, ws, viterbi, e->prop.multiProcessorCount * 8, e->stream);
+}
 static int run_viterbi(ckm_engine *e, const ckm_models *m, FilterParams &p, bool packed, DevBuf &grp) {
   int rc;
   if (packed) {
-    const int nm = (int)m->models.size();
-    const size_t nchunks = (size_t)p.in_cap / VITP_CHUNK + nm + 1;
-    const size_t words = 4 * (size_t)nm + 16 + ((size_t)p.in_cap + 1) / 2 * 2;
-    if ((rc = grp.alloc(sizeof(int32_t) * words + sizeof(int2) * nchunks))) return rc;
-    int32_t *ws = grp.as<int32_t>();
-    p.vit_cls_chunks = ws + 4 * (size_t)nm;
-    p.vit_idx = p.vit_cls_chunks + 16;
-    p.vit_chunks = reinterpret_cast<int2 *>(ws + words);
-    p.vit_work = e->d_counters + CTR_VWORK;
-    if ((rc = launch_vit_group(p, nm, ws, e->prop.multiProcessorCount * 8, e->stream))) return rc;
+    if ((rc = group_pairs(e, m, p, true, e->d_counters + CTR_VWORK, grp))) return rc;
     if ((rc = per_class<FilterParams>(e, p, launch_vitp, 8, nullptr, 0))) return rc;
     e->stats.kernel_launches += 3;
     p.in = p.redo; p.in_count = p.redo_count; p.in_cap = p.redo_cap;
@@ -300,7 +329,7 @@
   return per_class(e, p, launch_vit2, 8, launch_vit, 4);
 }
 struct Stage2 {
-  DevBuf a, b, redo, vgrp;
+  DevBuf a, b, redo, grp;
   int32_t cap = 0;
 };
 static int run_stage2(ckm_engine *e, const SearchKnobs &k, const ckm_models *m, const ckm_seqdb *db, ActiveMasks &am, Stage1 &s1, Stage2 &s2,
@@ -322,13 +351,14 @@
   CKM_CUDA(cudaEventRecord(e->ev[EV_VIT], st));
   p.in = s2.a.as<Candidate>(); p.in_count = e->d_counters + CTR_BIAS; p.in_cap = s2.cap;
   p.out = s2.b.as<Candidate>(); p.out_count = e->d_counters + CTR_VIT; p.out_cap = s2.cap;
-  if ((rc = run_viterbi(e, m, p, k.vitp, s2.vgrp))) return rc;
+  if ((rc = run_viterbi(e, m, p, k.vitp, s2.grp))) return rc;
   CKM_CUDA(cudaEventRecord(e->ev[EV_FWD], st));
   p.in = s2.b.as<Candidate>(); p.in_count = e->d_counters + CTR_VIT; p.in_cap = s2.cap;
   p.out = s2.a.as<Candidate>(); p.out_count = e->d_counters + CTR_FWD; p.out_cap = s2.cap;
+  if (p.use_blk && (rc = group_pairs(e, m, p, false, e->d_counters + CTR_FWORK, s2.grp))) return rc;
   if ((rc = per_class(e, p, launch_fwd2, 8, launch_fwd, 4, true))) return rc;
   CKM_CUDA(cudaEventRecord(e->ev[EV_CASCADE_END], st));
-  e->stats.kernel_launches += 3 + (k.vitp ? N_BLK_CLASSES : 0) + (p.use_blk ? 2 * N_BLK_CLASSES : 0);
+  e->stats.kernel_launches += 3 + (k.vitp ? N_BLK_CLASSES : 0) + (p.use_blk ? 2 * N_BLK_CLASSES + 3 : 0);
   return CKM_OK;
 }
 
@@ -345,25 +375,36 @@
   int rc;
   std::vector<int64_t> need(ev.size());
   std::vector<int8_t> ecls(ev.size());
+  std::vector<int32_t> emodel(ev.size());
   for (size_t i = 0; i < ev.size(); ++i) {
     const PairWork &pw = pairs[ev[i].pair];
     need[i] = envelope_need(m, pw, ev[i], p.use_blk != 0);
     ecls[i] = (int8_t)cls_of(m->models[pw.model].M, p.use_blk != 0);
-  }
+    emodel[i] = pw.model;
+  }
+  auto grouped = [](int c) { return c < N_BLK_CLASSES && blk_env_grouped(BLK_Q[c]); };
   budget = std::max<int64_t>(budget, *std::max_element(need.begin(), need.end()));
-  if ((rc = d_ev.alloc(sizeof(Envelope) * ev.size())) || (rc = d_ord.alloc(sizeof(int32_t) * ev.size()))) return rc;
+  const size_t chunk_off = (ev.size() + 1) / 2 * 2;
+  if ((rc = d_ev.alloc(sizeof(Envelope) * ev.size())) || (rc = d_ord.alloc(sizeof(int32_t) * (chunk_off + 2 * ev.size() + N_BLK_CLASSES + 1)))) return rc;
   std::vector<int32_t> eorder(ev.size());
   for (size_t w0 = 0, w1; w0 < ev.size(); w0 = w1) {
     int64_t tot = 0;
     for (w1 = w0; w1 < ev.size() && (w1 == w0 || tot + need[w1] <= budget); ++w1) { ev[w1].scratch_off = tot; tot += need[w1]; }
     if (sizeof(float) * (size_t)tot > scratch.bytes && (rc = scratch.alloc(sizeof(float) * (size_t)tot))) return rc;
+    e->stats.n_env_waves++;
     for (size_t i = w0; i < w1; ++i) eorder[i] = (int32_t)i;
-    std::stable_sort(eorder.begin() + w0, eorder.begin() + w1, [&](int32_t a, int32_t b) { return ecls[a] != ecls[b] ? ecls[a] > ecls[b] : need[a] > need[b]; });
+    std::stable_sort(eorder.begin() + w0, eorder.begin() + w1, [&](int32_t a, int32_t b) {
+      if (ecls[a] != ecls[b]) return ecls[a] > ecls[b];
+      if (grouped(ecls[a]) && emodel[a] != emodel[b]) return emodel[a] < emodel[b];
+      return need[a] > need[b]; });
     CKM_CUDA(cudaMemcpyAsync(d_ev.as<Envelope>() + w0, ev.data() + w0, sizeof(Envelope) * (w1 - w0), cudaMemcpyHostToDevice, st));
     CKM_CUDA(cudaMemcpyAsync(d_ord.as<int32_t>() + w0, eorder.data() + w0, sizeof(int32_t) * (w1 - w0), cudaMemcpyHostToDevice, st));
     p.envs = d_ev.as<Envelope>(); p.env_order = d_ord.as<int32_t>(); p.scratch = scratch.as<float>();
+    RunChunks rch{};
     if ((rc = launch_class_runs(e, eorder, ecls, w0, w1, [&](int c, int32_t b0, int32_t b1, int grid, cudaStream_t s) -> int {
-          p.env_begin = b0; p.env_end = b1; return c < N_BLK_CLASSES ? launch_envelopes2(p, c, grid, s) : launch_envelopes(p, grid, s); }))) return rc;
+          p.env_begin = b0; p.env_end = b1; p.chunks = rch.chunks; p.nchunks = rch.n; p.chunk_cursor = rch.cursor;
+          return c < N_BLK_CLASSES ? launch_envelopes2(p, c, grid, s) : launch_envelopes(p, grid, s); },
+          +grouped, &emodel, d_ord.as<int32_t>() + chunk_off, &rch))) return rc;
     CKM_CUDA(cudaStreamSynchronize(st));
     if (w1 < ev.size() || !leave_last) { if ((rc = fan_in(e))) return rc; CKM_CUDA(cudaStreamSynchronize(st)); }
   }
@@ -465,6 +506,7 @@
   tr.mark("regions kernels");
   if (nreg > region_cap) { set_error("region queue overflow"); return CKM_ECAPACITY; }
   D.regs.resize((size_t)nreg);
+  e->stats.n_regions = nreg;
   if (nreg) CKM_CUDA(cudaMemcpy(D.regs.data(), D.dregions.p, sizeof(Region) * D.regs.size(), cudaMemcpyDeviceToHost));
   std::sort(D.regs.begin(), D.regs.end(), [](const Region &a, const Region &b) { return a.pair != b.pair ? a.pair < b.pair : a.i < b.i; });
   tr.mark("regions sorted");
@@ -492,6 +534,7 @@
     nslots += n; pw.ndom_slots += n;
   }
   D.doms.assign((size_t)nslots, DomainOut{});
+  e->stats.n_envelopes = (int64_t)envs1.size(); e->stats.n_env_waves = 0;
   if (nslots == 0) return CKM_OK;
   if ((rc = D.ddoms.alloc(sizeof(DomainOut) * (size_t)nslots)) || (rc = D.dhits.alloc(sizeof(HitOut) * pairs.size()))) return rc;
   CKM_CUDA(cudaMemsetAsync(D.ddoms.p, 0, sizeof(DomainOut) * (size_t)nslots, st));
@@ -529,6 +572,7 @@
       return CKM_OK;
     }
     for (size_t mi = 0; mi < multi_idx.size(); ++mi) {
+      e->stats.n_envelopes += (int64_t)multi_envs[mi].size();
       int c = 0;
       for (Envelope en : multi_envs[mi]) { en.slot = reg_slot[multi_idx[mi]] + c++; envs2.push_back(en); }
     }
@@ -547,6 +591,7 @@
 static int run_domain_phase(ckm_engine *e, const SearchKnobs &k, const ckm_models *m, std::vector<PairWork> &pairs, DomainStage &D, Trace &tr) {
   std::vector<int> multi_idx;
   for (int r = 0; r < (int)D.regs.size(); ++r) if (D.regs[r].multi) multi_idx.push_back(r);
+  e->stats.n_multi_regions = (int64_t)multi_idx.size();
   std::vector<EnsembleCaps> caps(multi_idx.size(), ENS_DEFAULT_CAPS);
   D.hout.assign(pairs.size(), HitOut{});
   for (int pass = 0; pass < DOMAIN_PASSES; ++pass) {
diff --git a/checkm_b200/csrc/stages.hpp b/checkm_b200/csrc/stages.hpp
--- a/checkm_b200/csrc/stages.hpp
+++ b/checkm_b200/csrc/stages.hpp
@@ -67,7 +67,7 @@
   const uint4 *twb; const uint32_t *rwb; const float4 *tfb; const float *rfb;
   const uint4 *twp; const uint32_t *rwp;
   Candidate *redo; int32_t *redo_count; int32_t redo_cap;
-  int32_t *vit_idx; int2 *vit_chunks; int32_t *vit_cls_chunks; int32_t *vit_work;
+  int32_t *grp_idx; int2 *grp_chunks; int32_t *grp_cls_chunks; int32_t *grp_work;
   const Candidate *in; const int32_t *in_count; int32_t in_cap;
   Candidate *out; int32_t *out_count; int32_t out_cap;
   int32_t row_elems;
@@ -81,6 +81,7 @@
 constexpr int N_BLK_CLASSES = 10;
 constexpr int BLK_Q[N_BLK_CLASSES] = {2, 4, 6, 8, 12, 16, 20, 24, 28, 32};
 constexpr bool blk_tsmem(int q) { return q >= 12; }
+__host__ __device__ constexpr bool blk_env_grouped(int q) { return q >= 20; }
 __host__ __device__ constexpr int vq_of(int M) { return M <= 256 ? 2 * ((M + 63) / 64) : M <= 1024 ? 4 * ((M + 127) / 128) : 0; }
 __host__ __device__ constexpr int blk_class(int vq) { return vq == 0 ? N_BLK_CLASSES : (vq <= 8 ? vq / 2 - 1 : vq / 4 + 1); }
 constexpr bool blk_table_ok(int c = 0) {
@@ -111,8 +112,8 @@
 
 int launch_vit2(const FilterParams &p, int cls, int grid, cudaStream_t st);
 int launch_vitp(const FilterParams &p, int cls, int grid, cudaStream_t st);
-constexpr int VITP_CHUNK = 64;
-int launch_vit_group(const FilterParams &p, int32_t nmodels, int32_t *ws, int grid, cudaStream_t st);
+constexpr int GROUP_CHUNK = 64;
+int launch_group(const FilterParams &p, int32_t nmodels, int32_t *ws, bool viterbi, int grid, cudaStream_t st);
 int launch_all_pairs(Candidate *out, int32_t *count, const int32_t *slot_model, int32_t nslots, int32_t nseq, cudaStream_t st);
 int launch_fwd(const FilterParams &p, int grid, cudaStream_t st);
 
@@ -143,6 +144,7 @@
   int32_t *trace;
   Region *regions; int32_t *region_count; int32_t region_cap;
   const Envelope *envs; const int32_t *env_order; int32_t env_begin, env_end;
+  const int2 *chunks; int32_t nchunks; int32_t *chunk_cursor;
   float *scratch;
   DomainOut *doms; HitOut *hits;
   const float *logsum_tbl;
diff --git a/include/ckm.h b/include/ckm.h
--- a/include/ckm.h
+++ b/include/ckm.h
@@ -61,6 +61,8 @@
   int64_t n_vit_redo;
   int64_t n_msv_exact;
   int64_t n_queue_retries;
+  int64_t n_regions, n_multi_regions;
+  int64_t n_envelopes, n_env_waves;
 } ckm_stats;
 
 typedef struct {
```
